# experimental-design/everest

Measured on AMD Instinct MI355X. Metric: QnehviStrategy.ask() candidates/sec + GP posterior ms, n=512 d=6 m=5, higher is better.
Workload: dtype f64; 1 GPU; full QnehviStrategy.ask() of BASELINE configs[3] (config 4): DTLZ2(d=6,m=5), n_train=512, S=256 MC samples, 1024 raw Sobol candidates + 20 L-BFGS-B restarts, q=1; value = (raw + optimiser evaluations x batch) / ask wall time, SURVEY.md §8(d); n_train=512, d=6, m=5, mc_samples=256, raw_samples=1024, restarts=20, batch_limit=20, parallelism=1 rank

## Files before the change

everest_amd/_native.py:

```python
from __future__ import annotations

import ctypes
import os
from ctypes import POINTER, c_char_p, c_double, c_int, c_longlong, c_void_p

import torch

_HERE = os.path.dirname(os.path.abspath(__file__))
LIB_PATH = os.environ.get("EVR_LIB_PATH") or os.path.join(_HERE, "_lib", "libeverest_amd.so")

c_double_p = c_void_p
c_int_p = c_void_p


class NativeLibraryError(RuntimeError):
    pass


class EvrQnehviState(ctypes.Structure):
    _fields_ = [
        ("n", c_int), ("nb", c_int), ("S", c_int), ("m", c_int),
        ("c", c_void_p), ("ym", c_void_p), ("ys", c_void_p), ("kxx", c_void_p),
        ("zq", c_void_p), ("obj_a", c_void_p), ("obj_b", c_void_p),
        ("cell_lo", c_void_p), ("cell_hi", c_void_p), ("cell_off", c_void_p), ("max_cells", c_int),
        ("cell_keys", c_void_p), ("cell_pts", c_void_p), ("cell_rank0", c_void_p), ("pts_stride", c_int),
        ("grp_off", c_void_p), ("grp_keys", c_void_p), ("grp_rank", c_void_p), ("grp_box", c_void_p),
        ("sorted_lo", c_void_p), ("max_groups", c_int), ("scan_counters", c_void_p), ("no_h", c_int),
        ("log_hvi", c_int), ("tau_relu", c_double), ("tau_max", c_double),
    ]


class EvrQnehviModel(ctypes.Structure):
    _fields_ = [
        ("n", c_int), ("d", c_int), ("kind", c_int),
        ("Xn", c_void_p), ("lengthscales", c_void_p), ("shift", c_void_p), ("scale", c_void_p), ("M", c_void_p),
    ]


class EvrQnGeneral(ctypes.Structure):
    _fields_ = [
        ("q", c_int), ("m_obj", c_int),
        ("obj_out", c_void_p), ("obj_kind", c_void_p), ("obj_p0", c_void_p), ("obj_p1", c_void_p),
        ("n_con", c_int),
        ("con_out", c_void_p), ("con_sign", c_void_p), ("con_thr", c_void_p), ("con_eta", c_void_p),
        ("zq", c_void_p),
    ]

class EvrNei(ctypes.Structure):
    _fields_ = [
        ("log", c_int), ("tau_relu", c_double), ("tau_max", c_double), ("best", c_void_p), ("best_stride", c_int),
    ]


class EvrSobo(ctypes.Structure):
    _fields_ = [
        ("log", c_int), ("tau_relu", c_double), ("tau_max", c_double), ("best", c_void_p), ("best_stride", c_int),
        ("n_term", c_int),
        ("term_out", c_void_p), ("term_kind", c_void_p), ("term_w", c_void_p), ("term_p0", c_void_p),
        ("term_p1", c_void_p), ("term_p2", c_void_p),
        ("n_con", c_int),
        ("con_out", c_void_p), ("con_sign", c_void_p), ("con_thr", c_void_p), ("con_eta", c_void_p),
    ]


class EvrParego(ctypes.Structure):
    _fields_ = [
        ("log", c_int), ("tau_relu", c_double), ("tau_max", c_double), ("best", c_void_p), ("best_stride", c_int),
        ("alpha", c_double), ("n_term", c_int),
        ("term_out", c_void_p), ("term_kind", c_void_p), ("term_p0", c_void_p), ("term_p1", c_void_p),
        ("term_a", c_void_p), ("term_b", c_void_p),
        ("n_con", c_int),
        ("con_out", c_void_p), ("con_sign", c_void_p), ("con_thr", c_void_p), ("con_eta", c_void_p),
    ]


class EvrMult(ctypes.Structure):
    _fields_ = [
        ("log", c_int), ("tau_relu", c_double), ("tau_max", c_double), ("best", c_void_p), ("best_stride", c_int),
        ("n_fac", c_int),
        ("fac_out", c_void_p), ("fac_kind", c_void_p), ("fac_w", c_void_p), ("fac_p0", c_void_p),
        ("fac_p1", c_void_p), ("fac_p2", c_void_p),
        ("n_add", c_int),
        ("add_out", c_void_p), ("add_kind", c_void_p), ("add_w", c_void_p), ("add_p0", c_void_p),
        ("add_p1", c_void_p), ("add_p2", c_void_p),
    ]


class EvrReward(ctypes.Structure):
    _fields_ = [
        ("mode", c_int), ("ucb_scale", c_double), ("tau", c_double), ("best", c_void_p),
        ("infeasible_cost", c_double), ("n_term", c_int),
        ("term_out", c_void_p), ("term_kind", c_void_p), ("term_w", c_void_p), ("term_p0", c_void_p),
        ("term_p1", c_void_p), ("term_p2", c_void_p),
        ("n_con", c_int),
        ("con_out", c_void_p), ("con_sign", c_void_p), ("con_thr", c_void_p), ("con_eta", c_void_p),
    ]


_SIGS = {
    "evr_version": ([], c_int),
    "evr_last_error": ([], c_char_p),
    "evr_device_arch": ([c_int, c_char_p, c_int], c_int),
    "evr_stream_sync": ([c_void_p], c_int),
    "evr_kernel_matrix": ([c_void_p, c_int, c_int, c_int, c_int, c_int] + [c_void_p] * 10, c_int),
    "evr_kernel_cross_grad": ([c_void_p, c_int, c_int, c_int, c_int, c_int] + [c_void_p] * 11, c_int),
    "evr_kernel_cross_grad_workspace_doubles": ([c_int, c_int, c_int], c_longlong),
    "evr_kernel_lengthscale_grad": ([c_void_p, c_int, c_int, c_int, c_int, c_void_p, c_void_p, c_void_p,
                                     c_void_p, c_void_p], c_int),
    "evr_gp_mll_terms": ([c_void_p, c_int, c_int] + [c_void_p] * 5, c_int),
    "evr_gemm_f64": ([c_void_p, c_int, c_int, c_int, c_int, c_int, c_double, c_void_p, c_int, c_longlong,
                      c_void_p, c_int, c_longlong, c_double, c_void_p, c_int, c_longlong, c_int], c_int),
    "evr_cholesky": ([c_void_p, c_int, c_int, c_void_p, c_int, c_longlong, c_void_p, c_int, c_longlong,
                      c_double, c_int, c_void_p, c_void_p], c_int),
    "evr_cholesky_inverse": ([c_void_p, c_int, c_int, c_void_p, c_int, c_longlong, c_void_p, c_int, c_longlong,
                              c_void_p, c_int, c_longlong, c_double, c_int, c_void_p, c_void_p], c_int),
    "evr_trsm_lower":([c_void_p, c_int, c_int, c_int, c_void_p, c_int, c_longlong, c_int, c_void_p, c_int,
                        c_longlong], c_int),
    "evr_tri_inv_lower": ([c_void_p, c_int, c_int, c_void_p, c_int, c_longlong, c_void_p, c_int, c_longlong],
                          c_int),
    "evr_gp_posterior_finalize": ([c_void_p, c_int, c_int, c_int] + [c_void_p] * 8, c_int),
    "evr_gp_posterior_workspace_doubles": ([c_int, c_int, c_int], c_longlong),
    "evr_gp_posterior": ([c_void_p, c_int, c_int, c_int, c_int, c_int] + [c_void_p] * 14, c_int),
    "evr_qnehvi_samples": ([c_void_p, POINTER(EvrQnehviState), c_int, c_void_p, c_void_p, c_void_p, c_void_p],
                           c_int),
    "evr_hvi_workspace_doubles": ([POINTER(EvrQnehviState), c_int, c_int], c_longlong),
    "evr_hvi_forward": ([c_void_p, POINTER(EvrQnehviState), c_int, c_void_p, c_void_p, c_void_p, c_void_p],
                        c_int),
    "evr_mean_over_samples": ([c_void_p, c_int, c_int, c_void_p, c_void_p], c_int),
    "evr_hvi_backward": ([c_void_p, POINTER(EvrQnehviState), c_int, c_void_p, c_void_p, c_void_p, c_void_p],
                         c_int),
    "evr_qnehvi_samples_backward": ([c_void_p, POINTER(EvrQnehviState), c_int, c_void_p, c_void_p, c_void_p,
                                     c_void_p], c_int),
    "evr_pareto_mask": ([c_void_p, c_int, c_int, c_int, c_void_p, c_void_p, c_int, c_void_p, c_void_p], c_int),
    "evr_objective_affine": ([c_void_p, c_int, c_int, c_int] + [c_void_p] * 5, c_int),
    "evr_qei": ([c_void_p, c_int, c_int, c_int, c_void_p, c_double, c_double, c_double, c_double, c_void_p,
                 c_double, c_double, c_double, c_void_p, c_void_p, c_void_p], c_int),
    "evr_scale_batched":([c_void_p, c_int, c_longlong, c_void_p, c_void_p], c_int),
    "evr_add_selection": ([c_void_p, c_int, c_int, c_int, c_void_p, c_void_p, c_void_p], c_int),
    "evr_box_decompose": ([c_int, c_int, c_int, c_void_p, c_longlong, c_longlong, c_longlong, c_void_p,
                           c_void_p, c_int, POINTER(c_void_p)], c_int),
    "evr_box_decompose_approx": ([c_int, c_int, c_int, c_void_p, c_longlong, c_longlong, c_longlong, c_void_p,
                                  c_void_p, c_double, c_int, POINTER(c_void_p)], c_int),
    "evr_cells_total": ([c_void_p], c_longlong),
    "evr_cells_copy": ([c_void_p, c_void_p, c_void_p, c_void_p], c_int),
    "evr_cells_free": ([c_void_p], None),
    "evr_box_device_limits": ([c_int, c_int, c_void_p, c_void_p], c_int),
    "evr_box_device_workspace_bytes": ([c_int, c_int, c_int, c_int], c_longlong),
    "evr_box_decompose_device": ([c_void_p, c_int, c_int, c_int, c_void_p, c_void_p, c_int, c_void_p, c_void_p,
                                  c_void_p], c_int),
    "evr_box_pack_keys_device": ([c_void_p, c_int, c_int, c_int, c_int, c_void_p, c_void_p, c_int, c_void_p,
                                  c_void_p, c_void_p], c_int),
    "evr_box_kd_pipeline": ([c_void_p, c_int, c_int, c_int, c_void_p, c_void_p, c_int] + [c_void_p] * 8
                            + [c_int] + [c_void_p] * 6, c_int),
    "evr_cells_from_keys": ([c_void_p, c_int, c_int, c_int, c_void_p, c_int] + [c_void_p] * 5, c_int),
    "evr_hvi_forward_backward": ([c_void_p, POINTER(EvrQnehviState), c_int] + [c_void_p] * 6, c_int),
    "evr_hvi_restart_fb_applies": ([POINTER(EvrQnehviState), c_int], c_int),
    "evr_hvi_scan_limits": ([c_int, c_int], c_int),
    "evr_hvi_restart_fb": ([c_void_p, POINTER(EvrQnehviState), c_int] + [c_void_p] * 3, c_int),
    "evr_qnehvi_norms_rows": ([POINTER(EvrQnehviState)], c_int),
    "evr_qnehvi_project": ([c_void_p, POINTER(EvrQnehviState), c_int] + [c_void_p] * 5, c_int),
    "evr_qnehvi_project_workspace_doubles": ([POINTER(EvrQnehviState), c_int], c_longlong),
    "evr_qnehvi_samples_norms": ([c_void_p, POINTER(EvrQnehviState), c_int] + [c_void_p] * 5, c_int),
    "evr_qnehvi_project_backward": ([c_void_p, POINTER(EvrQnehviState), c_int] + [c_void_p] * 6, c_int),
    "evr_qnehvi_project_backward_workspace_doubles": ([POINTER(EvrQnehviState), c_int], c_longlong),
    "evr_qnehvi_plan_workspace_bytes": ([POINTER(EvrQnehviState), POINTER(EvrQnehviModel), c_int, c_int],
                                        c_longlong),
    "evr_qnehvi_plan_create": ([c_void_p, POINTER(EvrQnehviState), POINTER(EvrQnehviModel), c_int, c_int, c_void_p,
                               c_void_p, c_void_p, c_void_p, c_int, POINTER(c_void_p)], c_int),
    "evr_qnehvi_plan_run": ([c_void_p, c_void_p], c_int),
    "evr_qnehvi_small_applies": ([POINTER(EvrQnehviState), c_int, c_int], c_int),
    "evr_qnehvi_small_workspace_doubles": ([POINTER(EvrQnehviState), c_int, c_int, c_int], ctypes.c_longlong),
    "evr_qnehvi_small_forward": ([c_void_p, POINTER(EvrQnehviState), POINTER(EvrQnehviModel), c_int, c_void_p,
                                  c_void_p, c_void_p], c_int),
    "evr_qnehvi_small_samples": ([c_void_p, POINTER(EvrQnehviState), c_int, c_void_p, c_void_p, c_void_p, c_void_p,
                                  c_void_p], c_int),
    "evr_qnehvi_small_backward": ([c_void_p, POINTER(EvrQnehviState), POINTER(EvrQnehviModel), c_int, c_void_p,
                                   c_void_p, c_void_p, c_void_p, c_void_p, c_void_p], c_int),
    "evr_mll_plan_create": ([c_void_p, c_int, c_int, c_int, c_int, c_void_p, c_void_p, c_void_p], c_int),
    "evr_mll_plan_eval": ([c_void_p, c_void_p, c_void_p, c_void_p], c_int),
    "evr_mll_plan_destroy": ([c_void_p], None),
    "evr_mll_fit_rounds": ([c_void_p, c_void_p, c_void_p] + [c_void_p] * 7 + [c_int, c_int, c_void_p, c_void_p,
                                                                             c_void_p], c_int),
    "evr_mll_assemble": ([c_int, c_int, c_int] + [c_void_p] * 6, c_int),
    "evr_kernel_matrix_members": ([c_void_p, c_int, c_int, c_int, c_int] + [c_void_p] * 5, c_int),
    "evr_kernel_lengthscale_grad_members": ([c_void_p, c_int, c_int, c_int, c_int] + [c_void_p] * 5, c_int),
    "evr_mll_plan_create_members": ([c_void_p, c_int, c_int, c_int, c_int] + [c_void_p] * 4, c_int),
    "evr_mll_assemble_members": ([c_int, c_void_p, c_int] + [c_void_p] * 6, c_int),
    "evr_lbfgsb_advance": ([c_void_p, c_double] + [c_void_p] * 6 + [c_int, c_int], c_int),
    "evr_qnehvi_plan_eval_host": ([c_void_p, c_void_p, c_void_p, c_void_p], c_int),
    "evr_qnehvi_plan_destroy": ([c_void_p], None),
    "evr_lbfgsb_create": ([c_int, c_int, c_void_p, c_void_p, c_double, c_double, c_int, POINTER(c_void_p)], c_int),
    "evr_lbfgsb_start": ([c_void_p, c_void_p, c_void_p], c_int),
    "evr_lbfgsb_step": ([c_void_p, c_double, c_void_p, c_void_p], c_int),
    "evr_lbfgsb_stats": ([c_void_p, c_void_p, c_void_p, c_void_p, c_void_p], None),
    "evr_lbfgsb_destroy": ([c_void_p], None),
    "evr_hit_and_run": ([c_int, c_int, c_void_p, c_void_p, c_int, c_void_p, c_void_p, c_longlong, ctypes.c_ulonglong,
                         c_longlong, c_longlong, c_void_p], c_int),
    "evr_qnehvi_plan_minimize": ([c_void_p, c_void_p, c_void_p, c_void_p, c_void_p, c_int, c_int, c_double,
                                  c_double, c_int, c_int, c_void_p, c_void_p, c_void_p], c_int),
    "evr_qng_workspace_doubles": ([POINTER(EvrQnehviState), POINTER(EvrQnehviState), POINTER(EvrQnGeneral),
                                   POINTER(EvrQnehviModel), c_int, c_int], c_longlong),
    "evr_qng_eval": ([c_void_p, POINTER(EvrQnehviState), POINTER(EvrQnehviState), POINTER(EvrQnGeneral),
                      POINTER(EvrQnehviModel), c_int] + [c_void_p] * 5, c_int),
    "evr_qlog_workspace_doubles": ([POINTER(EvrQnehviState), POINTER(EvrQnehviState), POINTER(EvrQnGeneral),
                                    POINTER(EvrQnehviModel), c_int, c_int], ctypes.c_longlong),
    "evr_qlog_eval": ([c_void_p, POINTER(EvrQnehviState), POINTER(EvrQnehviState), POINTER(EvrQnGeneral),
                       POINTER(EvrQnehviModel), c_int] + [c_void_p] * 5, c_int),
    "evr_nei_scan": ([c_void_p, c_int, c_int, c_int, c_int, c_void_p, c_void_p, c_int, c_double, c_double, c_double,
                      c_double, c_void_p, c_void_p, c_void_p, c_void_p], c_int),
    "evr_qnei_workspace_doubles": ([POINTER(EvrQnehviState), POINTER(EvrQnGeneral), POINTER(EvrQnehviModel), c_int,
                                    c_int], c_longlong),
    "evr_qnei_eval": ([c_void_p, POINTER(EvrQnehviState), POINTER(EvrQnGeneral), POINTER(EvrQnehviModel),
                       POINTER(EvrNei), c_int] + [c_void_p] * 5, c_int),
    "evr_sobo_scan": ([c_void_p, c_int, c_int, c_int, c_int, POINTER(EvrSobo)] + [c_void_p] * 5, c_int),
    "evr_qsobo_workspace_doubles": ([POINTER(EvrQnehviState), POINTER(EvrQnGeneral), POINTER(EvrQnehviModel), c_int,
                                     c_int], c_longlong),
    "evr_qsobo_eval": ([c_void_p, POINTER(EvrQnehviState), POINTER(EvrQnGeneral), POINTER(EvrQnehviModel),
                        POINTER(EvrSobo), c_int] + [c_void_p] * 5, c_int),
    "evr_parego_scan": ([c_void_p, c_int, c_int, c_int, c_int, POINTER(EvrParego)] + [c_void_p] * 5, c_int),
    "evr_qparego_workspace_doubles": ([POINTER(EvrQnehviState), POINTER(EvrQnGeneral), POINTER(EvrQnehviModel),
                                       c_int, c_int], c_longlong),
    "evr_qparego_eval": ([c_void_p, POINTER(EvrQnehviState), POINTER(EvrQnGeneral), POINTER(EvrQnehviModel),
                          POINTER(EvrParego), c_int] + [c_void_p] * 5, c_int),
    "evr_mult_scan": ([c_void_p, c_int, c_int, c_int, c_int, POINTER(EvrMult)] + [c_void_p] * 5, c_int),
    "evr_qmult_workspace_doubles": ([POINTER(EvrQnehviState), POINTER(EvrQnGeneral), POINTER(EvrQnehviModel),
                                     c_int, c_int], c_longlong),
    "evr_qmult_eval": ([c_void_p, POINTER(EvrQnehviState), POINTER(EvrQnGeneral), POINTER(EvrQnehviModel),
                        POINTER(EvrMult), c_int] + [c_void_p] * 5, c_int),
    "evr_reward_scan": ([c_void_p, c_int, c_int, c_int, c_int, POINTER(EvrReward)] + [c_void_p] * 5, c_int),
    "evr_qreward_workspace_doubles": ([POINTER(EvrQnehviState), POINTER(EvrQnGeneral), POINTER(EvrQnehviModel),
                                       c_int, c_int], c_longlong),
    "evr_qreward_eval": ([c_void_p, POINTER(EvrQnehviState), POINTER(EvrQnGeneral), POINTER(EvrQnehviModel),
                          POINTER(EvrReward), c_int] + [c_void_p] * 5, c_int),
    "evr_nipv_reduce": ([c_void_p] + [c_int] * 7 + [c_void_p] * 2 + [c_int] + [c_void_p] * 13, c_int),
    "evr_mixed_kernel_matrix": ([c_void_p] + [c_int] * 6 + [c_void_p] * 7, c_int),
    "evr_mixed_kernel_param_grad": ([c_void_p] + [c_int] * 5 + [c_void_p] * 6, c_int),
    "evr_objective_general": ([c_void_p, c_int, c_int, c_int, POINTER(EvrQnGeneral)] + [c_void_p] * 4, c_int),
    "evr_objective_weights": ([c_void_p, c_int, c_int, POINTER(EvrQnGeneral)] + [c_void_p] * 3, c_int),
    "evr_cells_kd_limits": ([c_int, c_int, c_int, c_void_p], c_int),
    "evr_cells_kd_order_device": ([c_void_p, c_int, c_int, c_int, c_void_p, c_void_p, c_int] + [c_void_p] * 7,
                                  c_int),
    "evr_sobol_scramble": ([c_int, ctypes.c_ulonglong, c_void_p, c_void_p], c_int),
    "evr_sobol_scramble_range": ([c_int, ctypes.c_ulonglong, c_int, c_int, c_void_p, c_void_p], c_int),
    "evr_sobol_stream_words": ([c_int], ctypes.c_longlong),
    "evr_sobol_stream_create": ([ctypes.c_ulonglong, ctypes.c_longlong, c_void_p], c_int),
    "evr_sobol_scramble_stream": ([c_void_p, c_int, c_int, c_int, c_void_p, c_void_p], c_int),
    "evr_sobol_stream_destroy": ([c_void_p], None),
    "evr_sobol_normal": ([c_void_p, c_int, c_int, c_int, c_void_p, c_void_p, c_int, c_int, c_void_p], c_int),
}

EXPORTED_SYMBOLS = tuple(_SIGS)

_lib = None


def load() -> ctypes.CDLL:
    global _lib
    if _lib is not None:
        return _lib
    if not os.path.exists(LIB_PATH):
        raise NativeLibraryError(
            f"everest_amd native library not found at {LIB_PATH}; build it with "
            "`python -c 'import __graft_entry__ as g; g.build()'` (hipcc --offload-arch=gfx950)."
        )
    lib = ctypes.CDLL(LIB_PATH, mode=ctypes.RTLD_GLOBAL)
    for name, (args, res) in _SIGS.items():
        fn = getattr(lib, name)
        fn.argtypes = args
        fn.restype = res
    _lib = lib
    return lib


def check(status: int, what: str = ""):
    if status != 0:
        msg = load().evr_last_error().decode(errors="replace")
        raise RuntimeError(f"everest_amd {what} failed (status {status}): {msg}")


def call(name: str, *args):
    lib = load()
    check(getattr(lib, name)(*args), name)
```

everest_amd/acquisition.py:

```python
from __future__ import annotations

import ctypes
import math
import os
import warnings
from dataclasses import dataclass
from typing import Optional, Sequence

import numpy as np
import torch

from . import _native, ops
from .gp import GPBatch


def sobol_base_samples(S: int, n_points: int, m: int, seed: int, device, scrambled=None) -> torch.Tensor:
    return ops.sobol_normal(S, n_points * m, seed, device, layout=1, m=m, scrambled=scrambled)


_SCRAMBLE_POOL = None


def _prefetch_scramble(dim: int, seed: int, d0: int = 0, nd: Optional[int] = None):
    global _SCRAMBLE_POOL
    nd = dim - d0 if nd is None else nd
    if nd <= 0:
        return None
    key = (int(dim), int(seed), int(d0), int(nd))
    fut = _PREFETCHED.pop(key, None)
    if fut is not None:
        return fut
    if _SCRAMBLE_POOL is None:
        from concurrent.futures import ThreadPoolExecutor

        _SCRAMBLE_POOL = ThreadPoolExecutor(max_workers=3, thread_name_prefix="evr-sobol")
    return _SCRAMBLE_POOL.submit(ops.sobol_scramble, dim, seed, d0, nd)


_PREFETCHED = {}


def prefetch_scramble(dim: int, seed: int, d0: int = 0, nd: Optional[int] = None) -> None:
    nd = dim - d0 if nd is None else nd
    key = (int(dim), int(seed), int(d0), int(nd))
    if nd <= 0 or key in _PREFETCHED:
        return
    while len(_PREFETCHED) >= 8:
        _PREFETCHED.pop(next(iter(_PREFETCHED)))
    _PREFETCHED[key] = _prefetch_scramble(dim, seed, d0, nd)


def _submit(fn, *args):
    global _SCRAMBLE_POOL
    if _SCRAMBLE_POOL is None:
        from concurrent.futures import ThreadPoolExecutor

        _SCRAMBLE_POOL = ThreadPoolExecutor(max_workers=3, thread_name_prefix="evr-sobol")
    return _SCRAMBLE_POOL.submit(fn, *args)


def _prefetch_from_stream(fut_stream, dim: int, d0: int = 0, nd: Optional[int] = None):
    nd = dim - d0 if nd is None else nd
    if nd <= 0:
        return None
    return _submit(lambda: fut_stream.result().scramble(dim, d0, nd))


def _result(fut):
    return None if fut is None else fut.result()


def _host_threads() -> int:
    v = os.environ.get("EVR_HOST_THREADS") or os.environ.get("OMP_NUM_THREADS")
    try:
        return max(1, int(v)) if v else min(16, os.cpu_count() or 1)
    except ValueError:
        return 1


def _single_cell(ref: torch.Tensor, S: int, m: int) -> ops.Cells:
    dev = ref.device
    return ops.Cells(torch.arange(S + 1, dtype=torch.int32, device=dev), np.ones(S, dtype=np.int64), m,
                     lo=ref.unsqueeze(0).repeat(S, 1).contiguous(),
                     hi=torch.full((S, m), math.inf, dtype=torch.float64, device=dev))


def _decompose(O: torch.Tensor, ref: torch.Tensor, box_device=None, kd_scan=None, num_threads=None,
               alpha: float = 0.0):
    m, P, _ = O.shape
    dev = O.device
    approx = alpha > 0.0 and m > 2
    if approx and box_device:
        raise ValueError("the device box decomposition is exact only (alpha = 0)")
    if not approx and (box_device if box_device is not None else
                       ops.box_device_supported(P, m) and ops.hvi_scan_supported(P + m, m)):
        kd_built = False
        try:
            if kd_scan is False or os.environ.get("EVR_BOX_PIPELINE", "1") == "0":
                cells = ops.box_decompose_device(O, ref)
            else:
                cells, kd_built = ops.box_decompose_kd_device(O, ref, want_kd=True)
        except ops.BoxCapacityError as e:
            if box_device:
                raise
            warnings.warn(f"{e}; using the exact host partition", RuntimeWarning)
            cells = None
        if cells is not None:
            path = "device"
            if kd_built:
                path = "device+kd"
            elif kd_scan if kd_scan is not None else ops.kd_supported(cells):
                ops.cells_kd_order(cells)
                path = "device+kd"
            elif kd_scan is None:
                warnings.warn(f"{int(cells.counts.max())} cells in one sample exceed the sparse kd scan's limit; "
                              "using the dense tiled scan (~10x slower)", RuntimeWarning)
            return cells, path
    elif not approx and box_device is None:
        warnings.warn(f"{P} points x {m} objectives exceed the device box decomposition's limits; "
                      "using the host partition", RuntimeWarning)
    mask, _ = ops.pareto_mask(O, ref, dedup=True)
    lo, hi, off = ops.box_decompose(O.cpu().numpy(), ref.cpu().numpy(), mask.cpu().numpy(),
                                    num_threads or _host_threads(), layout="jis", alpha=alpha if approx else 0.0)
    f64 = dict(dtype=torch.float64, device=dev)
    return ops.Cells(torch.as_tensor(off, dtype=torch.int32, device=dev), np.diff(off), m,
                     lo=torch.as_tensor(lo, **f64), hi=torch.as_tensor(hi, **f64)), \
        ("host-approx" if approx else "host")


_BOX_POOL = None
_SIDE_STREAMS = {}


def _decompose_async(O: torch.Tensor, ref: torch.Tensor, *args):
    global _BOX_POOL
    if os.environ.get("EVR_BOX_OVERLAP", "1") == "0" or not O.is_cuda:
        res = _decompose(O, ref, *args)
        return lambda: res
    dev = O.device
    main = torch.cuda.current_stream(dev)
    side = _SIDE_STREAMS.get(dev)
    if side is None:
        side = _SIDE_STREAMS[dev] = torch.cuda.Stream(dev)
    ready = torch.cuda.Event()
    ready.record(main)
    O.record_stream(side)
    ref.record_stream(side)
    if _BOX_POOL is None:
        from concurrent.futures import ThreadPoolExecutor

        _BOX_POOL = ThreadPoolExecutor(max_workers=1, thread_name_prefix="evr-box")

    def job():
        with torch.cuda.device(dev), torch.cuda.stream(side):
            side.wait_event(ready)
            return _decompose(O, ref, *args)

    fut = _BOX_POOL.submit(job)

    def join():
        cells, path = fut.result()
        main.wait_stream(side)
        ts = [cells.off, cells.lo, cells.hi, cells.keys, cells.pts, cells.rank0]
        if cells.kd is not None:
            kd = cells.kd
            ts += [kd.goff, kd.keys, kd.rank, kd.box, kd.sorted_lo]
        for t in ts:
            if isinstance(t, torch.Tensor) and t.is_cuda:
                t.record_stream(main)
        return cells, path

    return join


def _make_spec(m: int, obj_a, obj_b, objective, constraints) -> ops.GeneralSpec:
    if objective is None:
        a = np.asarray(obj_a, dtype=np.float64).reshape(-1)
        b = np.asarray(obj_b, dtype=np.float64).reshape(-1)
        if a.shape[0] != m or b.shape[0] != m:
            raise ValueError(f"obj_a / obj_b need one entry per model output ({m})")
        objective = [(j, ops.OBJ_AFFINE, a[j], b[j]) for j in range(m)]
    return ops.GeneralSpec(m, objective, constraints or ())


def _fast_affine(spec: ops.GeneralSpec, m: int, dev):
    f64 = dict(dtype=torch.float64, device=dev)
    if spec.affine_identity:
        return (torch.tensor([o[2] for o in spec.objectives], **f64),
                torch.tensor([o[3] for o in spec.objectives], **f64))
    return torch.ones(m, **f64), torch.zeros(m, **f64)


@dataclass
class ConstructionStats:
    n_train: int
    n_base: int
    total_cells: int
    max_cells: int
    prune_probs: Optional[np.ndarray] = None


class _BoxHviAcqf:

    @property
    def ref_point(self) -> torch.Tensor:
        return self.ref

    @property
    def constraints(self) -> list:
        return list(self.spec.constraints)

    @property
    def eta(self) -> Optional[torch.Tensor]:
        cs = self.spec.constraints
        if not cs:
            return None
        e = torch.tensor([c[3] for c in cs], dtype=torch.float64)
        return e[0] if len(set(c[3] for c in cs)) == 1 else e

    def _use_log_scan(self, tau_relu: float, tau_max: float):
        if not (tau_relu > 0 and tau_max > 0):
            raise ValueError("tau_relu and tau_max must be positive")
        lo, hi = self.cells.explicit()

        def logify(src):
            st = _native.EvrQnehviState.from_buffer_copy(src)
            st.cell_lo, st.cell_hi = lo.data_ptr(), hi.data_ptr()
            st.log_hvi, st.tau_relu, st.tau_max = 1, float(tau_relu), float(tau_max)
            return st
        self._log_cells = (lo, hi)
        self.state_scan = logify(self.state_scan)
        self.state = logify(self.state)
        if self.spec.affine_identity:
            self.state_model = self.state
        self.tau_relu, self.tau_max = float(tau_relu), float(tau_max)
        self.log_acqf = True
        self._plans = {}

    @property
    def supports_plan(self) -> bool:
        return self.spec.affine_identity and self._pending_rows() is None

    def _init_general(self, spec: ops.GeneralSpec, cells, nk: int, nb_rows: int, no_h: bool = False):
        gp, m = self.gp, self.m
        self.spec = spec
        self._zq_cache = {}
        if spec.affine_identity:
            self.state_model = self.state_scan = self.state
        else:
            ones = torch.ones(max(m, spec.m_obj), dtype=torch.float64, device=self.dev)
            self._dummy = (ones, torch.zeros_like(ones))
            self.state_model = ops.make_state(nk, nb_rows, self.S, m, gp.const, gp.ym, gp.ys, gp.kxx, self.zq,
                                              ones, ones, cells, no_h=no_h)
            self.state_scan = ops.make_state(nk, nb_rows, self.S, spec.m_obj, ones, ones, ones, ones, self.zq,
                                             ones, ones, cells, no_h=no_h)

    def _zq(self, q: int) -> torch.Tensor:
        z = self._zq_cache.get(q)
        if z is None:
            z = self._draw_zq(q).to(dtype=torch.float64, device=self.dev).reshape(self.S, q, self.m).contiguous()
            self._zq_cache[q] = z
        return z

    def set_new_point_samples(self, q: int, z: torch.Tensor):
        self._zq_cache[int(q)] = z.to(dtype=torch.float64, device=self.dev).reshape(self.S, q, self.m).contiguous()

    def _pending_rows(self) -> Optional[torch.Tensor]:
        return None

    def _general(self, X: torch.Tensor, backward: bool, gout: Optional[torch.Tensor] = None):
        b, q, d = X.shape
        Xp = self._pending_rows()
        qq = q
        if Xp is not None:
            X = torch.cat([X, Xp.unsqueeze(0).expand(b, Xp.shape[0], d)], 1)
            qq = X.shape[1]
        if qq > ops.QNG_MAX_Q:
            raise ValueError(f"joint batch of {qq} points (q + pending) exceeds the device limit of {ops.QNG_MAX_Q} "
                             f"(the inclusion-exclusion runs over all 2^q - 1 subsets)")
        g = self.spec.struct(qq, self._zq(qq))
        ev = ops.qlog_eval if getattr(self, "log_acqf", False) else ops.qng_eval
        acq, dX = ev(self.state_model, self.state_scan, g, self.model, X.reshape(b * qq, d).contiguous(),
                     backward, gout)
        if dX is not None:
            dX = dX.view(b, qq, d)[:, :q].contiguous()
        return acq, dX

    def _device_tensors(self):
        out, seen = [], set()

        def walk(v, depth=0):
            if isinstance(v, torch.Tensor):
                if v.device.type == "cuda" and id(v) not in seen:
                    seen.add(id(v))
                    out.append(v)
            elif depth >= 4 or id(v) in seen:
                return
            elif isinstance(v, (list, tuple)):
                for x in v:
                    walk(x, depth + 1)
            elif isinstance(v, dict):
                for x in v.values():
                    walk(x, depth + 1)
            elif type(v).__module__.startswith("everest_amd") and hasattr(v, "__dict__"):
                seen.add(id(v))
                for k, x in vars(v).items():
                    if k not in ("_torch_acqs", "_plans"):
                        walk(x, depth + 1)
        walk(self)
        return out

    def _torch_acq(self, q: int, fast: bool):
        from . import torch_ops

        torch_ops.load()
        cache = self.__dict__.setdefault("_torch_acqs", {})
        acq = cache.get(fast)
        if acq is None:
            def raw(st):
                return torch.frombuffer(bytearray(bytes(st)), dtype=torch.uint8)
            stm = self.state if fast else self.state_model
            sth = self.state if fast else self.state_scan
            acq = torch.classes.everest_amd.QnehviAcq(raw(stm), raw(sth), raw(self.model), bool(fast),
                                                      bool(getattr(self, "log_acqf", False)), self._device_tensors())
            cache[fast] = acq
        done = self.__dict__.setdefault("_torch_general_q", set())
        if not fast and q not in done:
            spec = self.spec
            oo, ok, p0, p1 = spec._arrs
            cons = spec.constraints
            co = torch.tensor([c[0] for c in cons], dtype=torch.int32)
            cs, ct, ce = (torch.tensor([c[k] for c in cons], dtype=torch.float64) for k in (1, 2, 3))
            acq.set_general(int(q), torch.from_numpy(oo), torch.from_numpy(ok), torch.from_numpy(p0),
                            torch.from_numpy(p1), co, cs, ct, ce, self._zq(q))
            done.add(q)
        return acq

    def __call__(self, X: torch.Tensor) -> torch.Tensor:
        from .torch_ops import QnehviFunction

        X3, _ = self._split(X)
        if self._fast(X3):
            return QnehviFunction.apply(X3[:, 0].contiguous(), self._torch_acq(1, True))
        Xp = self._pending_rows()
        if Xp is not None:
            X3 = torch.cat([X3, Xp.unsqueeze(0).expand(X3.shape[0], Xp.shape[0], X3.shape[2])], 1)
        if X3.shape[1] > ops.QNG_MAX_Q:
            raise ValueError(f"joint batch of {X3.shape[1]} points (q + pending) exceeds the device limit of "
                             f"{ops.QNG_MAX_Q} (the inclusion-exclusion runs over all 2^q - 1 subsets)")
        return QnehviFunction.apply(X3.contiguous(), self._torch_acq(X3.shape[1], False))

    def _split(self, X: torch.Tensor):
        X = X.to(device=self.dev, dtype=torch.float64)
        if X.dim() == 2:
            return X.unsqueeze(1), True
        if X.dim() != 3:
            raise ValueError(f"candidates must be b x d or b x q x d, got {tuple(X.shape)}")
        return X, False

    def _fast(self, X3: torch.Tensor) -> bool:
        return X3.shape[1] == 1 and self.supports_plan and self._pending_rows() is None

    def plan(self, b: int, backward: bool) -> ops.QnehviPlan:
        if not self.supports_plan:
            raise NotImplementedError("the native plan covers q = 1 with affine objectives on every output")
        key = (int(b), bool(backward))
        p = self._plans.get(key)
        if p is None:
            if len(self._plans) >= 8:
                self._plans.pop(next(iter(self._plans)))
            p = ops.QnehviPlan(self.state, self.model, int(b), bool(backward), self.dev,
                               graph=os.environ.get("EVR_GRAPH", "1") != "0")
            self._plans[key] = p
        return p

    def forward(self, X: torch.Tensor, return_cache: bool = False):
        if return_cache:
            return self.forward_ops(X, return_cache=True)
        X3, _ = self._split(X)
        if not self._fast(X3):
            return self._general(X3, False)[0]
        p = self.plan(X3.shape[0], False)
        p.X.copy_(X3[:, 0])
        p.run()
        return p.acq.clone()

    def forward_backward(self, X: torch.Tensor, gout: Optional[torch.Tensor] = None):
        X3, flat = self._split(X)
        if not self._fast(X3):
            acq, dX = self._general(X3, True, gout)
            return acq, (dX[:, 0] if flat else dX)
        if gout is not None:
            acq, dX = self.forward_backward_ops(X3[:, 0], gout)
            return acq, (dX if flat else dX.unsqueeze(1))
        p = self.plan(X3.shape[0], True)
        p.X.copy_(X3[:, 0])
        p.run()
        return p.acq.clone(), (p.dX.clone() if flat else p.dX.clone().unsqueeze(1))

    def eval_host(self, x: np.ndarray, backward: bool):
        b = x.shape[0]
        if x.ndim == 2 and self.supports_plan and self._pending_rows() is None:
            out = self.plan(b, backward).run_host(x)
            acq = out[:b].copy()
            return acq, (out[b:].reshape(b, -1).copy() if backward else None)
        Xt = torch.as_tensor(x, dtype=torch.float64, device=self.dev)
        if backward:
            a, g = self.forward_backward(Xt)
            return a.cpu().numpy(), g.cpu().numpy()
        return self.forward(Xt).cpu().numpy(), None

    def _cross(self, X: torch.Tensor) -> torch.Tensor:
        gp = self.gp
        return ops.kernel_matrix(self.Xk, X, gp.ls, gp.kind, shift2=gp.lo, scale2=gp.inv_range)

    def forward_ops(self, X: torch.Tensor, return_cache: bool = False):
        X = X.to(device=self.dev, dtype=torch.float64).contiguous()
        b = X.shape[0]
        Kx = self._cross(X)
        R, P = ops.qnehvi_project(self.state, self.M, Kx, b)
        G, L22, flags = ops.qnehvi_samples_norms(self.state, R, P, b)
        acq = ops.hvi_forward(self.state, G, b, flags)
        if return_cache:
            return acq, (X, R, G, L22, flags)
        return acq

    def forward_backward_ops(self, X: torch.Tensor, gout: Optional[torch.Tensor] = None):
        X = X.to(device=self.dev, dtype=torch.float64).contiguous()
        b = X.shape[0]
        Kx = self._cross(X)
        R, P = ops.qnehvi_project(self.state, self.M, Kx, b)
        G, L22, flags = ops.qnehvi_samples_norms(self.state, R, P, b)
        acq, dG = ops.hvi_forward_backward(self.state, G, b, flags, gout)
        dKx = ops.qnehvi_project_backward(self.state, self.M, R, L22, dG, b)
        gp = self.gp
        dX = ops.kernel_cross_grad(self.Xk, X, gp.ls, dKx, gp.kind, shift2=gp.lo, scale2=gp.inv_range)
        return acq, dX


class QNEHVI(_BoxHviAcqf):

    def __init__(self, gp: GPBatch, X_train_raw: np.ndarray, X_baseline_raw: np.ndarray, ref_point, obj_a, obj_b,
                 S: int = 512, sampler_seed: int = 0, prune_baseline: bool = True, prune_seed: int = 0,
                 prune_samples: int = 2048, max_frac: float = 1.0, z_prune: Optional[torch.Tensor] = None,
                 z_base_full: Optional[torch.Tensor] = None, z_new_full: Optional[torch.Tensor] = None,
                 num_threads: Optional[int] = None, box_device: Optional[bool] = None,
                 kd_scan: Optional[bool] = None, X_pending_raw: Optional[np.ndarray] = None,
                 root: Optional[str] = None, objective=None, constraints=(), alpha: float = 0.0):
        dev = gp.device
        self.gp = gp
        self.dev = dev
        m = gp.B
        n = gp.n
        self.m, self.n, self.S = m, n, int(S)
        f64 = dict(dtype=torch.float64, device=dev)
        spec = _make_spec(m, obj_a, obj_b, objective, constraints)
        self.spec = spec
        self.ref = torch.as_tensor(np.asarray(ref_point, dtype=np.float64), **f64)
        if self.ref.numel() != spec.m_obj:
# ... 944 lines not shown
```

everest_amd/csrc/box_device.hip:

```cpp
#include <algorithm>
#include <cmath>
#include <cstdlib>

#include "common.hpp"
#include "../../include/everest_amd.h"

namespace evr {

constexpr int BD_THREADS = 1024;
constexpr unsigned long long BD_DEAD = ~0ull;
constexpr int BD_LDS_BYTES = 160 * 1024 - 2048;
constexpr int BD_STG = 256;

struct BdLayout {
  long long cap;
  int n, m;
  size_t off_lub, off_buf, off_aidx, off_pts, off_inv0, off_nf, bytes;
};

static BdLayout bd_layout(int S, int n, int m, int cap) {
  BdLayout L;
  L.cap = cap;
  L.n = n;
  L.m = m;
  size_t o = 0;
  auto take = [&](size_t b) {
    size_t r = o;
    o += (b + 255) & ~(size_t)255;
    return r;
  };
  L.off_lub = take(sizeof(unsigned long long) * (size_t)S * cap);
  L.off_buf = take(sizeof(unsigned long long) * (size_t)S * cap);
  L.off_aidx = take(sizeof(int) * (size_t)S * cap);
  L.off_pts = take(sizeof(double) * (size_t)S * (n + m) * m);
  L.off_inv0 = take(sizeof(int) * (size_t)S * (n + m));
  L.off_nf = take(sizeof(int) * (size_t)S);
  L.bytes = o;
  return L;
}

static size_t bd_lds_fixed(int n, int m) {
  return sizeof(double) * ((size_t)n * m + (size_t)(n + m) * m) + sizeof(int) * (size_t)(4 * n + 2 * m + 8);
}

template <typename Ptr>
__device__ void bd_bitonic(Ptr a, int P2) {
  for (int k = 2; k <= P2; k <<= 1) {
    for (int j = k >> 1; j > 0; j >>= 1) {
      for (int i = threadIdx.x; i < P2; i += BD_THREADS) {
        const int l = i ^ j;
        if (l > i) {
          const unsigned long long x = a[i], y = a[l];
          const bool up = (i & k) == 0;
          if ((x > y) == up) {
            a[i] = y;
            a[l] = x;
          }
        }
      }
      __syncthreads();
    }
  }
}

template <int M, bool LS>
__global__ __launch_bounds__(BD_THREADS) void bd_build_kernel(int S, int n, const double* __restrict__ obj,
                                                              const double* __restrict__ ref, int cap, int sortcap,
                                                              unsigned char* __restrict__ ws, BdLayout Lo,
                                                              int* __restrict__ counts, int* __restrict__ status,
                                                              int* hmap) {
  using K = CellKey<M>;
  extern __shared__ __align__(16) unsigned char smem[];
  const int s = blockIdx.x, tid = threadIdx.x;
  double* raw = (double*)smem;
  double* pt = raw + (size_t)n * M;
  int* flag = (int*)(pt + (size_t)(n + M) * M);
  int* pos = flag + n;
  int* inv0 = pos + n;
  int* rank = inv0 + n + M;
  unsigned long long* sbuf = (unsigned long long*)(((uintptr_t)(rank + n + M) + 15) & ~(uintptr_t)15);
  unsigned long long* stg = sbuf + sortcap;
  int* astg = (int*)(stg + BD_STG);
  __shared__ int sh_nf, sh_nA, sh_nNew, sh_cnt, sh_err;

  unsigned long long* lub = LS ? sbuf : (unsigned long long*)(ws + Lo.off_lub) + (size_t)s * cap;
  unsigned long long* buf = (unsigned long long*)(ws + Lo.off_buf) + (size_t)s * cap;
  int* aidx = (int*)(ws + Lo.off_aidx) + (size_t)s * cap;
  double* gpts = (double*)(ws + Lo.off_pts) + (size_t)s * (n + M) * M;
  int* ginv0 = (int*)(ws + Lo.off_inv0) + (size_t)s * (n + M);

  for (int e = tid; e < n * M; e += BD_THREADS) {
    const int i = e / M, j = e - i * M;
    raw[e] = -obj[((size_t)j * n + i) * S + s];
  }
  if (tid == 0) sh_err = 0;
  __syncthreads();
  for (int i = tid; i < n; i += BD_THREADS) {
    bool keep = true;
#pragma unroll
    for (int j = 0; j < M; ++j) keep &= raw[i * M + j] < -ref[j];
    for (int k = 0; k < n && keep; ++k) {
      if (k == i) continue;
      bool cand = true, le = true, lt = false, eq = true;
#pragma unroll
      for (int j = 0; j < M; ++j) {
        const double v = raw[k * M + j], w = raw[i * M + j];
        cand &= v < -ref[j];
        le &= v <= w;
        lt |= v < w;
        eq &= v == w;
      }
      if (cand && ((le && lt) || (eq && k < i))) keep = false;
    }
    flag[i] = keep ? 1 : 0;
  }
  __syncthreads();
  if (tid == 0) {
    int c = 0;
    for (int i = 0; i < n; ++i) {
      pos[i] = c;
      c += flag[i];
    }
    sh_nf = c;
  }
  __syncthreads();
  const int nf = sh_nf;
  for (int e = tid; e < n * M; e += BD_THREADS) {
    const int i = e / M;
    if (flag[i]) pt[pos[i] * M + (e - i * M)] = raw[e];
  }
  for (int e = tid; e < M * M; e += BD_THREADS) {
    const int k = e / M, j = e - k * M;
    pt[(nf + k) * M + j] = (j == k) ? -ref[k] : -INFINITY;
  }
  __syncthreads();
  for (int i = tid; i <= nf; i += BD_THREADS) {
    const double v = pt[i * M];
    int r = 0;
    for (int k = 0; k <= nf; ++k) {
      const double w = pt[k * M];
      r += (w > v) || (w == v && k < i);
    }
    inv0[r] = i;
    rank[i] = r;
  }
  __syncthreads();

  int Kend = 1, holes = 0;
  if (tid == 0) {
    unsigned long long k0 = 0;
    k0 = K::set(k0, 0, rank[nf]);
    for (int j = 1; j < M; ++j) k0 = K::set(k0, j, nf + j);
    lub[0] = k0;
  }
  __syncthreads();
  for (int p = 0; p < nf; ++p) {
    double z[M];
#pragma unroll
    for (int j = 0; j < M; ++j) z[j] = pt[p * M + j];
    if (tid == 0) {
      sh_nA = 0;
      sh_nNew = 0;
    }
    __syncthreads();
    for (int u = tid; u < Kend; u += BD_THREADS) {
      const unsigned long long key = lub[u];
      if (key == BD_DEAD) continue;
      bool dom = pt[inv0[K::field(key, 0)] * M] > z[0];
#pragma unroll
      for (int j = 1; j < M; ++j) dom &= pt[K::field(key, j) * M + j] > z[j];
      if (dom) {
        const int k = atomicAdd(&sh_nA, 1);
        if (LS && k < BD_STG) astg[k] = u;
        else aidx[k] = u;
      }
    }
    __syncthreads();
    const int nA = sh_nA;
    for (int t = tid; t < nA * M; t += BD_THREADS) {
      const int a = t / M, j = t - a * M;
      const unsigned long long key = lub[(LS && a < BD_STG) ? astg[a] : aidx[a]];
      double zmax = -INFINITY;
#pragma unroll
      for (int k = 0; k < M; ++k) {
        if (k == j) continue;
        const int pk = (k == 0) ? inv0[K::field(key, 0)] : K::field(key, k);
        zmax = fmax(zmax, pt[pk * M + j]);
      }
      if (z[j] >= zmax) {
        const int slot = atomicAdd(&sh_nNew, 1);
        if (slot < cap) {
          const unsigned long long nk = K::set(key, j, j == 0 ? rank[p] : p);
          if (LS && slot < BD_STG) stg[slot] = nk;
          else buf[slot] = nk;
        }
      }
    }
    __syncthreads();
    const int nNew = sh_nNew;
    if (Kend + (nNew > nA ? nNew - nA : 0) > cap || nNew > cap) {
      if (tid == 0) sh_err = 1;
      break;
    }
    const int top = nNew > nA ? nNew : nA;
    for (int i = tid; i < top; i += BD_THREADS) {
      const bool st = LS && i < BD_STG;
      if (i < nNew) {
        const int dst = (i < nA) ? (st ? astg[i] : aidx[i]) : Kend + (i - nA);
        lub[dst] = st ? stg[i] : buf[i];
      } else {
        lub[st ? astg[i] : aidx[i]] = BD_DEAD;
      }
    }
    if (nNew > nA) Kend += nNew - nA;
    else holes += nA - nNew;
    __syncthreads();
    if (holes > 256 && holes * 4 > Kend) {
      if (tid == 0) sh_cnt = 0;
      __syncthreads();
      for (int u = tid; u < Kend; u += BD_THREADS) {
        const unsigned long long key = lub[u];
        if (key != BD_DEAD) buf[atomicAdd(&sh_cnt, 1)] = key;
      }
      __syncthreads();
      const int cnt = sh_cnt;
      for (int u = tid; u < cnt; u += BD_THREADS) lub[u] = buf[u];
      Kend = cnt;
      holes = 0;
      __syncthreads();
    }
  }
  __syncthreads();
  if (sh_err) {
    if (tid == 0) {
      status[s] = 1;
      counts[s] = 0;
      if (hmap) {
        hmap[s] = 0;
        hmap[S + s] = 1;
      }
    }
    return;
  }

  if (tid == 0) sh_cnt = 0;
  __syncthreads();
  for (int u = tid; u < Kend; u += BD_THREADS) {
    const unsigned long long key = lub[u];
    if (key == BD_DEAD) continue;
    int P[M];
    P[0] = inv0[K::field(key, 0)];
#pragma unroll
    for (int j = 1; j < M; ++j) P[j] = K::field(key, j);
    bool ok = true;
#pragma unroll
    for (int j = 1; j < M; ++j) {
      double lo = -INFINITY;
#pragma unroll
      for (int k = 0; k < j; ++k) lo = fmax(lo, pt[P[k] * M + j]);
      ok &= pt[P[j] * M + j] > lo;
    }
    if (ok) buf[atomicAdd(&sh_cnt, 1)] = key;
  }
  __syncthreads();
  const int C = sh_cnt;
  int P2 = 1;
  while (P2 < C) P2 <<= 1;
  if (P2 <= sortcap) {
    for (int i = tid; i < P2; i += BD_THREADS) sbuf[i] = (i < C) ? buf[i] : BD_DEAD;
    __syncthreads();
    wg_bitonic<unsigned long long, BD_THREADS>(sbuf, P2);
    for (int i = tid; i < C; i += BD_THREADS) buf[i] = sbuf[i];
  } else {
    for (int i = C + tid; i < P2; i += BD_THREADS) buf[i] = BD_DEAD;
    __syncthreads();
    bd_bitonic(buf, P2);
  }
  for (int e = tid; e < (nf + M) * M; e += BD_THREADS) gpts[e] = pt[e];
  for (int r = tid; r <= nf; r += BD_THREADS) ginv0[r] = inv0[r];
  if (tid == 0) {
    counts[s] = C;
    status[s] = 0;
    ((int*)(ws + Lo.off_nf))[s] = nf;
    if (hmap) {
      hmap[s] = C;
      hmap[S + s] = 0;
    }
  }
}

template <int M>
__global__ __launch_bounds__(256) void cells_from_keys_kernel(int stride, const int* __restrict__ off,
                                                              const unsigned long long* __restrict__ keys,
                                                              const double* __restrict__ pts,
                                                              const int* __restrict__ rank0, double* __restrict__ lo,
                                                              double* __restrict__ hi) {
  using K = CellKey<M>;
  const int s = blockIdx.y;
  const int i = blockIdx.x * 256 + threadIdx.x;
  const int c0 = off[s], C = off[s + 1] - c0;
  if (i >= C) return;
  double l[M], h[M];
  K::decode(keys[c0 + i], pts + (size_t)s * stride * M, rank0 + (size_t)s * stride, l, h);
  const size_t o = (size_t)(c0 + i) * M;
#pragma unroll
  for (int j = 0; j < M; ++j) {
    lo[o + j] = l[j];
    hi[o + j] = h[j];
  }
}

template <int M>
__global__ __launch_bounds__(256) void bd_pack_keys_kernel(int S, int n, int cap, const unsigned char* __restrict__ ws,
                                                           BdLayout Lo, const int* __restrict__ off,
                                                           unsigned long long* __restrict__ keys,
                                                           double* __restrict__ pts, int* __restrict__ rank0) {
  const int s = blockIdx.y;
  const int i = blockIdx.x * 256 + threadIdx.x;
  const int c0 = off[s], C = off[s + 1] - c0;
  if (i < C) keys[c0 + i] = ((const unsigned long long*)(ws + Lo.off_buf))[(size_t)s * cap + i];
  if (blockIdx.x == 0) {
    const size_t np = (size_t)(n + M);
    const double* gp = (const double*)(ws + Lo.off_pts) + s * np * M;
    const int* gi = (const int*)(ws + Lo.off_inv0) + s * np;
    const size_t nv = (size_t)((const int*)(ws + Lo.off_nf))[s] + M;
    for (size_t e = threadIdx.x; e < np * M; e += 256) pts[s * np * M + e] = e < nv * M ? gp[e] : INFINITY;
    for (size_t e = threadIdx.x; e < np; e += 256) rank0[s * np + e] = e + M <= nv ? gi[e] : 0;
  }
}

}

using namespace evr;

#define EVR_BD_SWITCH(m, MACRO)                                                       \
  switch (m) {                                                                        \
    case 1: MACRO(1); break;                                                          \
    case 2: MACRO(2); break;                                                          \
    case 3: MACRO(3); break;                                                          \
    case 4: MACRO(4); break;                                                          \
    case 5: MACRO(5); break;                                                          \
    case 6: MACRO(6); break;                                                          \
    case 7: MACRO(7); break;                                                          \
    case 8: MACRO(8); break;                                                          \
    default: EVR_CHECK(false, "box decomposition: m=%d not supported (1..8)", m);     \
  }

extern "C" {

int evr_box_device_limits(int n, int m, int* max_points_out, long long* lds_bytes_out) {
  EVR_CHECK(m >= 1 && m <= 8 && n >= 0, "evr_box_device_limits: bad arguments");
  const long long idx_limit = (1ll << bd_field_bits(m)) - 2 - m;
  const size_t fixed = bd_lds_fixed(n, m);
  if (max_points_out) *max_points_out = (int)std::min<long long>(idx_limit, 1 << 20);
  if (lds_bytes_out) *lds_bytes_out = (long long)fixed;
  return (n <= idx_limit && fixed + 16 + 8 * 64 <= (size_t)BD_LDS_BYTES) ? 0 : 3;
}

long long evr_box_device_workspace_bytes(int S, int n, int m, int cap) {
  if (S < 1 || n < 0 || m < 1 || cap < 1) return 0;
  return (long long)bd_layout(S, n, m, cap).bytes;
}

static int box_decompose_launch(void* stream, int S, int n, int m, const double* obj, const double* ref, int cap,
                                void* work, int* counts, int* status, int* hmap);

int evr_box_decompose_device(void* stream, int S, int n, int m, const double* obj, const double* ref, int cap,
                             void* work, int* counts, int* status) {
  return box_decompose_launch(stream, S, n, m, obj, ref, cap, work, counts, status, nullptr);
}

static int box_decompose_launch(void* stream, int S, int n, int m, const double* obj, const double* ref, int cap,
                                void* work, int* counts, int* status, int* hmap) {
  EVR_CHECK(S >= 1 && n >= 1 && m >= 1 && m <= 8 && obj && ref && work && counts && status,
            "evr_box_decompose_device: bad arguments");
  EVR_CHECK(cap >= 2 && (cap & (cap - 1)) == 0, "evr_box_decompose_device: cap must be a power of two");
  EVR_CHECK(evr_box_device_limits(n, m, nullptr, nullptr) == 0,
            "evr_box_decompose_device: n=%d points x m=%d exceed the device limits", n, m);
  const BdLayout Lo = bd_layout(S, n, m, cap);
  const size_t fixed = bd_lds_fixed(n, m) + 16;
  auto sort_cap = [&](size_t fx) {
    int c = 1;
    while ((size_t)(c * 2) * 8 + fx <= (size_t)BD_LDS_BYTES && c * 2 <= cap) c *= 2;
    return c;
  };
  const size_t fixed_ls = fixed + (size_t)BD_STG * (8 + 4);
  const char* ev = std::getenv("EVR_BD_LDS");
  const bool ls = sort_cap(fixed_ls) >= cap && !(ev && ev[0] == '0');
  const int sortcap = ls ? cap : sort_cap(fixed);
  const size_t lds = (ls ? fixed_ls : fixed) + (size_t)sortcap * 8;
  hipStream_t s = (hipStream_t)stream;
#define L2(MM, LS_)                                                                                          \
  do {                                                                                                       \
    EVR_HIP(hipFuncSetAttribute((const void*)bd_build_kernel<MM, LS_>,                                      \
                                hipFuncAttributeMaxDynamicSharedMemorySize, (int)lds));                      \
    bd_build_kernel<MM, LS_><<<S, BD_THREADS, lds, s>>>(S, n, obj, ref, cap, sortcap, (unsigned char*)work, \
                                                        Lo, counts, status, hmap);                           \
  } while (0)
#define L(MM)            \
  if (ls) L2(MM, true);  \
  else L2(MM, false)
  EVR_BD_SWITCH(m, L);
#undef L
#undef L2
  EVR_LAUNCH_CHECK();
  return 0;
}

int evr_cells_from_keys(void* stream, int S, int m, int stride, const int* off, int max_cells,
                        const unsigned long long* keys, const double* pts, const int* rank0, double* lo,
                        double* hi) {
  EVR_CHECK(S >= 1 && m >= 1 && m <= 8 && stride > m && off && keys && pts && rank0 && lo && hi,
            "evr_cells_from_keys: bad arguments");
  if (max_cells <= 0) return 0;
  dim3 grid(cdiv(max_cells, 256), S);
  hipStream_t s = (hipStream_t)stream;
#define L(MM) cells_from_keys_kernel<MM><<<grid, 256, 0, s>>>(stride, off, keys, pts, rank0, lo, hi)
  EVR_BD_SWITCH(m, L);
#undef L
  EVR_LAUNCH_CHECK();
  return 0;
}

int evr_box_pack_keys_device(void* stream, int S, int n, int m, int cap, const void* work, const int* off,
                             int max_cells, unsigned long long* keys, double* pts, int* rank0) {
  EVR_CHECK(S >= 1 && n >= 1 && m >= 1 && m <= 8 && work && off && keys && pts && rank0,
            "evr_box_pack_keys_device: bad arguments");
  const BdLayout Lo = bd_layout(S, n, m, cap);
  dim3 grid(std::max(1, cdiv(max_cells, 256)), S);
  hipStream_t s = (hipStream_t)stream;
#define L(MM) \
  bd_pack_keys_kernel<MM><<<grid, 256, 0, s>>>(S, n, cap, (const unsigned char*)work, Lo, off, keys, pts, rank0)
  EVR_BD_SWITCH(m, L);
#undef L
  EVR_LAUNCH_CHECK();
  return 0;
}


int evr_box_kd_pipeline(void* stream, int S, int n, int m, const double* obj, const double* ref, int cap,
                        void* work, int* counts_dev, int* status_dev, int* off_dev, int* goff_dev,
                        unsigned long long* keys, double* pts, int* rank0, int want_kd, unsigned long long* okeys,
                        unsigned short* ork, unsigned short* ogb, double* osv, int* counts_host, int* info) {
  EVR_CHECK(S >= 1 && counts_dev && status_dev && off_dev && goff_dev && keys && pts && rank0 && counts_host &&
                info && (!want_kd || (okeys && ork && ogb && osv)),
            "evr_box_kd_pipeline: bad arguments");
  hipStream_t s = (hipStream_t)stream;
  thread_local int* stage = nullptr;
  thread_local int* stage_d = nullptr;
  thread_local size_t stage_n = 0;
  thread_local int stage_dev = -1;
  thread_local hipEvent_t copied = nullptr;
  if (copied) EVR_HIP(hipEventSynchronize(copied));
  int dev = 0;
  EVR_HIP(hipGetDevice(&dev));
  const size_t need = (size_t)4 * S + 2;
  if (stage_n < need || stage_dev != dev) {
    if (copied) {
      (void)hipEventDestroy(copied);
      copied = nullptr;
    }
    if (stage) (void)hipHostFree(stage);
    stage = stage_d = nullptr;
    stage_n = 0;
    stage_dev = -1;
    EVR_HIP(hipHostMalloc((void**)&stage, sizeof(int) * need, hipHostMallocMapped | hipHostMallocCoherent));
    EVR_HIP(hipHostGetDevicePointer((void**)&stage_d, stage, 0));
    stage_n = need;
    stage_dev = dev;
  }
  if (!copied) EVR_HIP(hipEventCreateWithFlags(&copied, hipEventDisableTiming));
  int* hc = stage;
  int* hs = stage + S;
  int* hoff = stage + 2 * S;
  int* hgoff = hoff + S + 1;
  if (int rc = box_decompose_launch(stream, S, n, m, obj, ref, cap, work, counts_dev, status_dev, stage_d)) return rc;
  EVR_HIP(hipStreamSynchronize(s));
  info[0] = info[1] = info[2] = 0;
  int maxc = 0;
  for (int i = 0; i < S; ++i) {
    counts_host[i] = hc[i];
    if (hs[i]) info[0] = 1;
    maxc = std::max(maxc, hc[i]);
  }
  info[2] = maxc;
  if (info[0]) return 0;
  long long c = 0, g = 0;
  for (int i = 0; i < S; ++i) {
    hoff[i] = (int)c;
    hgoff[i] = (int)g;
    c += hc[i];
    g += (hc[i] + 15) / 16;
  }
  hoff[S] = (int)c;
  hgoff[S] = (int)g;
  EVR_CHECK(c <= (long long)S * cap && c < 0x7FFFFFFFLL, "evr_box_kd_pipeline: %lld cells exceed the capacity", c);
  const int* moff = stage_d + 2 * S;
  const int* mgoff = moff + S + 1;
  if (int rc = evr_box_pack_keys_device(stream, S, n, m, cap, work, moff, maxc, keys, pts, rank0)) return rc;
  const int stride = n + m;
  if (want_kd && evr_cells_kd_limits(stride, m, maxc, nullptr) == 0) {
    if (int rc = evr_cells_kd_order_device(stream, S, m, stride, moff, mgoff, maxc, keys, pts, rank0, okeys, ork,
                                           ogb, osv))
      return rc;
    info[1] = 1;
  }
  EVR_HIP(hipMemcpyAsync(off_dev, hoff, sizeof(int) * (S + 1), hipMemcpyHostToDevice, s));
  EVR_HIP(hipMemcpyAsync(goff_dev, hgoff, sizeof(int) * (S + 1), hipMemcpyHostToDevice, s));
  EVR_HIP(hipEventRecord(copied, s));
  return 0;
}

}
```

everest_amd/csrc/qnehvi.hip:

```cpp
#include <algorithm>
#include <cstdlib>
#include <string>
#include "common.hpp"
#include "../../include/everest_amd.h"

namespace evr {

template <int BX>
__global__ __launch_bounds__(256) void qn_samples_kernel(int n, int nb, int S, int nh, int m, int b,
                                                         const double* __restrict__ R,
                                                         const double* __restrict__ cc,
                                                         const double* __restrict__ ym,
                                                         const double* __restrict__ ys,
                                                         const double* __restrict__ kxx,
                                                         const double* __restrict__ zq,
                                                         const double* __restrict__ oa,
                                                         const double* __restrict__ ob, double* __restrict__ G,
                                                         double* __restrict__ L22, int* __restrict__ flags) {
  constexpr int RY = 256 / BX;
  __shared__ double red[2][RY][BX];
  const int j = blockIdx.y;
  const int cx = threadIdx.x % BX, ry = threadIdx.x / BX;
  const int c = blockIdx.x * BX + cx;
  const bool live = c < b;
  const long long Rr = (long long)n + nb + nh + 1;
  const double* Rj = R + (size_t)j * Rr * b;
  double ssv = 0.0, ssw = 0.0;
  if (live) {
    for (int i = ry; i < n; i += RY) {
      const double v = Rj[(size_t)i * b + c];
      ssv = fma(v, v, ssv);
    }
    for (int i = n + ry; i < n + nb; i += RY) {
      const double v = Rj[(size_t)i * b + c];
      ssw = fma(v, v, ssw);
    }
  }
  red[0][ry][cx] = ssv;
  red[1][ry][cx] = ssw;
  __syncthreads();
  ssv = 0.0;
  ssw = 0.0;
#pragma unroll
  for (int g = 0; g < RY; ++g) {
    ssv += red[0][g][cx];
    ssw += red[1][g][cx];
  }
  if (!live) return;
  const double a = Rj[(size_t)(n + nb + nh) * b + c];
  const double s = ys[j];
  const double mu = ym[j] + s * (cc[j] + a);
  const double var = s * s * (kxx[j] - ssv);
  const double br = var - ssw;
  double l22 = nan("");
  int flag = 1;
  if (!isnan(br)) {
    for (int t = 0; t <= 6; ++t) {
      const double jit = (t == 0) ? 0.0 : 1e-8 * pow(10.0, (double)(t - 1));
      if (br + jit > 0.0) {
        l22 = sqrt(br + jit);
        flag = 0;
        break;
      }
    }
  }
  if (ry == 0) {
    L22[(size_t)j * b + c] = l22;
    flags[(size_t)j * b + c] = flag;
  }
  const double A = oa[j], B0 = ob[j];
  const double* h = Rj + (size_t)(n + nb) * b + c;
  for (int si = ry; si < S; si += RY) {
    const double y = (nh ? mu + h[(size_t)si * b] : mu) + l22 * zq[(size_t)si * m + j];
    G[((size_t)si * m + j) * b + c] = fma(A, y, B0);
  }
}

__global__ void mean_over_samples_kernel(int S, int b, const double* __restrict__ partial, double* __restrict__ acq) {
  const int c = blockIdx.x * blockDim.x + threadIdx.x;
  if (c >= b) return;
  double s = 0.0;
  for (int i = 0; i < S; ++i) s += partial[(size_t)i * b + c];
  acq[c] = s / (double)S;
}

template <int BX>
__global__ __launch_bounds__(256) void qn_samples_bwd_kernel(int n, int nb, int S, int nh, int m, int b,
                                                             const double* __restrict__ R,
                                                             const double* __restrict__ ys,
                                                             const double* __restrict__ zq,
                                                             const double* __restrict__ oa,
                                                             const double* __restrict__ L22,
                                                             const double* __restrict__ dG, double* __restrict__ gR) {
  constexpr int RY = 256 / BX;
  __shared__ double red[2][RY][BX];
  const int j = blockIdx.y;
  const int cx = threadIdx.x % BX, ry = threadIdx.x / BX;
  const int c = blockIdx.x * BX + cx;
  const bool live = c < b;
  const long long Rr = (long long)n + nb + nh + 1;
  const double* Rj = R + (size_t)j * Rr * b;
  double* gj = gR + (size_t)j * Rr * b;
  const double A = oa[j];
  double dmu = 0.0, dl = 0.0;
  if (live) {
    for (int si = ry; si < S; si += RY) {
      const double dy = A * dG[((size_t)si * m + j) * b + c];
      dmu += dy;
      dl = fma(dy, zq[(size_t)si * m + j], dl);
      if (nh) gj[(size_t)(n + nb + si) * b + c] = dy;
    }
  }
  red[0][ry][cx] = dmu;
  red[1][ry][cx] = dl;
  __syncthreads();
  dmu = 0.0;
  dl = 0.0;
#pragma unroll
  for (int g = 0; g < RY; ++g) {
    dmu += red[0][g][cx];
    dl += red[1][g][cx];
  }
  if (!live) return;
  const double s = ys[j];
  if (ry == 0) gj[(size_t)(n + nb + nh) * b + c] = s * dmu;
  const double l22 = L22[(size_t)j * b + c];
  const double dbr = dl / (2.0 * l22);
  const double dssv = -s * s * dbr;
  const double dssw = -dbr;
  for (int i = ry; i < n; i += RY) gj[(size_t)i * b + c] = 2.0 * Rj[(size_t)i * b + c] * dssv;
  for (int i = n + ry; i < n + nb; i += RY) gj[(size_t)i * b + c] = 2.0 * Rj[(size_t)i * b + c] * dssw;
}

template <int M>
__global__ void pareto_kernel(int S, int n, const double* __restrict__ O, const double* __restrict__ ref,
                              int dedup, unsigned char* __restrict__ mask, int* __restrict__ counts) {
  const int s = blockIdx.x * blockDim.x + threadIdx.x;
  const int i = blockIdx.y;
  if (s >= S) return;
  double yi[M];
  bool better = true;
#pragma unroll
  for (int j = 0; j < M; ++j) {
    yi[j] = O[((size_t)j * n + i) * S + s];
    better &= yi[j] > ref[j];
  }
  bool nd = better;
  for (int k = 0; k < n && nd; ++k) {
    if (k == i) continue;
    bool ge = true, gt = false, eq = true;
#pragma unroll
    for (int j = 0; j < M; ++j) {
      const double v = O[((size_t)j * n + k) * S + s];
      ge &= v >= yi[j];
      gt |= v > yi[j];
      eq &= v == yi[j];
    }
    if (ge && gt) nd = false;
    if (dedup && eq && k < i) nd = false;
  }
  if (mask) mask[(size_t)s * n + i] = nd ? 1 : 0;
  if (counts && nd) atomicAdd(&counts[i], 1);
}

template <int M>
__global__ __launch_bounds__(256) void pareto_lds_kernel(int S, int n, int SB, const double* __restrict__ O,
                                                         const double* __restrict__ ref, int dedup,
                                                         unsigned char* __restrict__ mask, int* __restrict__ counts) {
  extern __shared__ double pts[];
  const int s0 = blockIdx.x * SB, sb = min(SB, S - s0);
  const int tot = M * n * sb;
  for (int e = threadIdx.x; e < tot; e += 256) {
    const int j = e / (n * sb), rem = e - j * n * sb, k = rem / sb, ss = rem - k * sb;
    pts[((size_t)ss * n + k) * M + j] = O[((size_t)j * n + k) * S + s0 + ss];
  }
  double rj[M];
#pragma unroll
  for (int j = 0; j < M; ++j) rj[j] = ref[j];
  __syncthreads();
  for (int p = threadIdx.x; p < sb * n; p += 256) {
    const int ss = p / n, i = p - ss * n;
    const double* P = pts + (size_t)ss * n * M;
    double yi[M];
    bool better = true;
#pragma unroll
    for (int j = 0; j < M; ++j) {
      yi[j] = P[i * M + j];
      better &= yi[j] > rj[j];
    }
    bool nd = better;
    constexpr int U = 8;
    for (int k0 = 0; k0 < n && nd; k0 += U) {
      double v[U][M];
#pragma unroll
      for (int u = 0; u < U; ++u)
#pragma unroll
        for (int j = 0; j < M; ++j) v[u][j] = (k0 + u < n) ? P[(k0 + u) * M + j] : 0.0;
#pragma unroll
      for (int u = 0; u < U; ++u) {
        const int k = k0 + u;
        if (k >= n || k == i) continue;
        bool ge = true, gt = false, eq = true;
#pragma unroll
        for (int j = 0; j < M; ++j) {
          ge &= v[u][j] >= yi[j];
          gt |= v[u][j] > yi[j];
          eq &= v[u][j] == yi[j];
        }
        if (ge && gt) nd = false;
        if (dedup && eq && k < i) nd = false;
      }
    }
    if (mask) mask[(size_t)(s0 + ss) * n + i] = nd ? 1 : 0;
    if (counts && nd) atomicAdd(&counts[i], 1);
  }
}

template <int M>
__global__ __launch_bounds__(256) void pareto_f32_kernel(int S, int n, int npad, int SB, const double* __restrict__ O,
                                                         const double* __restrict__ ref, int dedup,
                                                         unsigned char* __restrict__ mask, int* __restrict__ counts) {
  extern __shared__ double pts[];
  float* ptf = reinterpret_cast<float*>(pts + (((size_t)SB * n * M + 1) & ~(size_t)1));
  const int s0 = blockIdx.x * SB, sb = min(SB, S - s0);
  const int tot = M * n * sb;
  for (int e = threadIdx.x; e < tot; e += 256) {
    const int j = e / (n * sb), rem = e - j * n * sb, k = rem / sb, ss = rem - k * sb;
    const double v = O[((size_t)j * n + k) * S + s0 + ss];
    pts[((size_t)ss * n + k) * M + j] = v;
    ptf[((size_t)ss * M + j) * npad + k] = (float)v;
  }
  for (int e = threadIdx.x; e < sb * M * (npad - n); e += 256) {
    const int r = e / (npad - n), k = n + (e - r * (npad - n));
    ptf[(size_t)r * npad + k] = -INFINITY;
  }
  double rj[M];
#pragma unroll
  for (int j = 0; j < M; ++j) rj[j] = ref[j];
  __syncthreads();
  for (int p = threadIdx.x; p < sb * n; p += 256) {
    const int ss = p / n, i = p - ss * n;
    const double* P = pts + (size_t)ss * n * M;
    const float* F = ptf + (size_t)ss * M * npad;
    double yi[M];
    float yf[M];
    bool better = true;
#pragma unroll
    for (int j = 0; j < M; ++j) {
      yi[j] = P[i * M + j];
      yf[j] = (float)yi[j];
      better &= yi[j] > rj[j];
    }
    bool nd = better;
    for (int k0 = 0; k0 < n && nd; k0 += 8) {
      float4 va[M], vb[M];
#pragma unroll
      for (int j = 0; j < M; ++j) {
        va[j] = *reinterpret_cast<const float4*>(F + (size_t)j * npad + k0);
        vb[j] = *reinterpret_cast<const float4*>(F + (size_t)j * npad + k0 + 4);
      }
      bool ge8[8];
#pragma unroll
      for (int u = 0; u < 8; ++u) ge8[u] = k0 + u != i && k0 + u < n;
#pragma unroll
      for (int j = 0; j < M; ++j) {
        ge8[0] &= va[j].x >= yf[j]; ge8[1] &= va[j].y >= yf[j];
        ge8[2] &= va[j].z >= yf[j]; ge8[3] &= va[j].w >= yf[j];
        ge8[4] &= vb[j].x >= yf[j]; ge8[5] &= vb[j].y >= yf[j];
        ge8[6] &= vb[j].z >= yf[j]; ge8[7] &= vb[j].w >= yf[j];
      }
      unsigned int cand = 0;
#pragma unroll
      for (int u = 0; u < 8; ++u) cand |= (unsigned int)ge8[u] << u;
      while (cand) {
        const int u = __builtin_ctz(cand);
        cand &= cand - 1;
        const int k = k0 + u;
        bool ge = true, gt = false, eq = true;
#pragma unroll
        for (int j = 0; j < M; ++j) {
          const double v = P[k * M + j];
          ge &= v >= yi[j];
          gt |= v > yi[j];
          eq &= v == yi[j];
        }
        if ((ge && gt) || (dedup && eq && k < i)) {
          nd = false;
          cand = 0;
        }
      }
    }
    if (mask) mask[(size_t)(s0 + ss) * n + i] = nd ? 1 : 0;
    if (counts && nd) atomicAdd(&counts[i], 1);
  }
}

__global__ void qei_kernel(int n, int b, int S, const double* __restrict__ R, double cc, double ym, double ys,
                           double kxx, const double* __restrict__ z, double oa, double ob, double best_f,
                           double* __restrict__ acq, double* __restrict__ gR, int* __restrict__ flags) {
  const int c = blockIdx.x * blockDim.x + threadIdx.x;
  if (c >= b) return;
  double ss = 0.0;
  for (int i = 0; i < n; ++i) {
    const double v = R[(size_t)i * b + c];
    ss = fma(v, v, ss);
  }
  const double mu = ym + ys * (cc + R[(size_t)n * b + c]);
  const double var = ys * ys * (kxx - ss);
  double sd = nan("");
  int flag = 1;
  if (!isnan(var)) {
    for (int t = 0; t <= 3; ++t) {
      const double jit = (t == 0) ? 0.0 : 1e-8 * pow(10.0, (double)(t - 1));
      if (var + jit > 0.0) {
        sd = sqrt(var + jit);
        flag = 0;
        break;
      }
    }
  }
  double tot = 0.0, dmu = 0.0, dsd = 0.0;
  for (int s = 0; s < S; ++s) {
    const double imp = oa * (mu + sd * z[s]) + ob - best_f;
    if (imp > 0.0) {
      tot += imp;
      dmu += oa;
      dsd += oa * z[s];
    }
  }
  acq[c] = tot / S;
  flags[c] = flag;
  if (gR) {
    dmu /= S;
    dsd /= S;
    const double dvar = dsd / (2.0 * sd);
    const double dss = -ys * ys * dvar;
    for (int i = 0; i < n; ++i) gR[(size_t)i * b + c] = 2.0 * R[(size_t)i * b + c] * dss;
    gR[(size_t)n * b + c] = ys * dmu;
  }
}

__global__ void scale_batched_kernel(long long per, const double* __restrict__ alpha, double* __restrict__ X) {
  const long long e = (long long)blockIdx.x * blockDim.x + threadIdx.x;
  if (e >= per) return;
  X[(size_t)blockIdx.y * per + e] *= alpha[blockIdx.y];
}

__global__ void add_selection_kernel(int nb, int n, const int* __restrict__ idx, const double* __restrict__ val,
                                     double* __restrict__ E) {
  const int r = blockIdx.x * blockDim.x + threadIdx.x;
  if (r >= nb) return;
  const int b = blockIdx.y;
  E[((size_t)b * nb + r) * n + idx[r]] += val ? val[b] : 1.0;
}

__global__ void objective_affine_kernel(int m, int n, int S, const double* __restrict__ Y, const double* __restrict__ mu,
                                        const double* __restrict__ a, const double* __restrict__ bb,
                                        double* __restrict__ O) {
  const long long e = (long long)blockIdx.x * blockDim.x + threadIdx.x;
  const long long tot = (long long)m * n * S;
  if (e >= tot) return;
  const int j = (int)(e / ((long long)n * S));
  const int i = (int)((e / S) % n);
  const double mv = mu ? mu[(size_t)j * n + i] : 0.0;
  O[e] = fma(a[j], Y[e] + mv, bb[j]);
}

}

using namespace evr;

#define EVR_DISPATCH_M(m, MACRO)                                                      \
  switch (m) {                                                                        \
    case 1: MACRO(1); break;                                                          \
    case 2: MACRO(2); break;                                                          \
    case 3: MACRO(3); break;                                                          \
    case 4: MACRO(4); break;                                                          \
    case 5: MACRO(5); break;                                                          \
    case 6: MACRO(6); break;                                                          \
    case 7: MACRO(7); break;                                                          \
    case 8: MACRO(8); break;                                                          \
    default: EVR_CHECK(false, "number of objectives m=%d not supported (1..8)", m);   \
  }

extern "C" {

int evr_qnehvi_samples(void* stream, const evr_qnehvi_state* st, int b, const double* R, double* G, double* L22,
                       int* flags) {
  EVR_CHECK(st && st->m >= 1 && st->S >= 1 && st->n >= 1 && st->nb >= 0, "evr_qnehvi_samples: bad state");
  if (b == 0) return 0;
  hipStream_t s = (hipStream_t)stream;
  if (b <= 256) {
    dim3 grid(cdiv(b, 16), st->m);
    qn_samples_kernel<16><<<grid, 256, 0, s>>>(st->n, st->nb, st->S, qn_nh(st), st->m, b, R, st->c, st->ym, st->ys, st->kxx,
                                               st->zq, st->obj_a, st->obj_b, G, L22, flags);
  } else {
    dim3 grid(cdiv(b, 64), st->m);
    qn_samples_kernel<64><<<grid, 256, 0, s>>>(st->n, st->nb, st->S, qn_nh(st), st->m, b, R, st->c, st->ym, st->ys, st->kxx,
                                               st->zq, st->obj_a, st->obj_b, G, L22, flags);
  }
  EVR_LAUNCH_CHECK();
  return 0;
}

int evr_mean_over_samples(void* stream, int S, int b, const double* partial, double* acq) {
  if (b == 0) return 0;
  mean_over_samples_kernel<<<cdiv(b, 256), 256, 0, (hipStream_t)stream>>>(S, b, partial, acq);
  EVR_LAUNCH_CHECK();
  return 0;
}

int evr_qnehvi_samples_backward(void* stream, const evr_qnehvi_state* st, int b, const double* R, const double* L22,
                                const double* dG, double* gR) {
  EVR_CHECK(st && st->m >= 1, "evr_qnehvi_samples_backward: bad state");
  if (b == 0) return 0;
  hipStream_t s = (hipStream_t)stream;
  if (b <= 256) {
    dim3 grid(cdiv(b, 16), st->m);
    qn_samples_bwd_kernel<16><<<grid, 256, 0, s>>>(st->n, st->nb, st->S, qn_nh(st), st->m, b, R, st->ys, st->zq, st->obj_a,
                                                   L22, dG, gR);
  } else {
    dim3 grid(cdiv(b, 64), st->m);
    qn_samples_bwd_kernel<64><<<grid, 256, 0, s>>>(st->n, st->nb, st->S, qn_nh(st), st->m, b, R, st->ys, st->zq, st->obj_a,
                                                   L22, dG, gR);
  }
  EVR_LAUNCH_CHECK();
  return 0;
}

int evr_pareto_mask(void* stream, int S, int n, int m, const double* O, const double* ref, int dedup,
                    unsigned char* mask, int* counts) {
  EVR_CHECK(S >= 1 && n >= 0, "evr_pareto_mask: bad sizes");
  if (n == 0) return 0;
  hipStream_t s = (hipStream_t)stream;
  constexpr size_t kLds = 96 * 1024;
  const size_t per = (size_t)n * m * sizeof(double);
  constexpr int f32_filter = 1;
  const int npad = (n + 7) & ~7;
  const size_t per2 = (size_t)n * m * sizeof(double) + (size_t)npad * m * sizeof(float);
  constexpr size_t kLds2 = 78 * 1024;
  if (f32_filter && per2 <= kLds2) {
    const int SB = (int)std::min<size_t>(4, kLds2 / per2);
    const size_t bytes = (((size_t)SB * n * m + 1) & ~(size_t)1) * sizeof(double) + (size_t)SB * npad * m * sizeof(float);
#define L(MM)                                                                                            \
  do {                                                                                                   \
    EVR_HIP(hipFuncSetAttribute((const void*)pareto_f32_kernel<MM>,                                       \
                                hipFuncAttributeMaxDynamicSharedMemorySize, (int)bytes));                \
    pareto_f32_kernel<MM><<<cdiv(S, SB), 256, bytes, s>>>(S, n, npad, SB, O, ref, dedup, mask, counts);  \
  } while (0)
    EVR_DISPATCH_M(m, L);
#undef L
  } else if (per <= kLds) {
    const int SB = (int)std::min<size_t>(4, kLds / per);
    const size_t bytes = per * SB;
#define L(MM)                                                                                            \
  do {                                                                                                   \
    EVR_HIP(hipFuncSetAttribute((const void*)pareto_lds_kernel<MM>,                                       \
                                hipFuncAttributeMaxDynamicSharedMemorySize, (int)bytes));                \
    pareto_lds_kernel<MM><<<cdiv(S, SB), 256, bytes, s>>>(S, n, SB, O, ref, dedup, mask, counts);       \
  } while (0)
    EVR_DISPATCH_M(m, L);
#undef L
  } else {
    dim3 grid(cdiv(S, 64), n);
#define L(MM) pareto_kernel<MM><<<grid, 64, 0, s>>>(S, n, O, ref, dedup, mask, counts)
    EVR_DISPATCH_M(m, L);
#undef L
  }
  EVR_LAUNCH_CHECK();
  return 0;
}

int evr_qei(void* stream, int n, int b, int S, const double* R, double c, double ym, double ys, double kxx,
            const double* z, double obj_a, double obj_b, double best_f, double* acq, double* gR, int* flags) {
  EVR_CHECK(n >= 1 && S >= 1, "evr_qei: bad sizes");
  if (b == 0) return 0;
  qei_kernel<<<cdiv(b, 256), 256, 0, (hipStream_t)stream>>>(n, b, S, R, c, ym, ys, kxx, z, obj_a, obj_b, best_f,
                                                            acq, gR, flags);
  EVR_LAUNCH_CHECK();
  return 0;
}

int evr_scale_batched(void* stream, int B, long long per, const double* alpha, double* X) {
  if (per == 0) return 0;
  dim3 grid(cdiv(per, 256), B);
  scale_batched_kernel<<<grid, 256, 0, (hipStream_t)stream>>>(per, alpha, X);
  EVR_LAUNCH_CHECK();
  return 0;
}

int evr_add_selection(void* stream, int B, int nb, int n, const int* idx, const double* val, double* E) {
  if (nb == 0) return 0;
  dim3 grid(cdiv(nb, 256), B);
  add_selection_kernel<<<grid, 256, 0, (hipStream_t)stream>>>(nb, n, idx, val, E);
  EVR_LAUNCH_CHECK();
  return 0;
}

int evr_objective_affine(void* stream, int m, int n, int S, const double* Y, const double* mu, const double* a,
                         const double* b, double* O) {
  const long long tot = (long long)m * n * S;
  if (tot == 0) return 0;
  objective_affine_kernel<<<cdiv(tot, 256), 256, 0, (hipStream_t)stream>>>(m, n, S, Y, mu, a, b, O);
  EVR_LAUNCH_CHECK();
  return 0;
}

}
```

everest_amd/ops.py:

```python
from __future__ import annotations

import ctypes
import math
import os
import warnings
from typing import Optional, Tuple

import numpy as np
import torch

from . import _native
from ._native import EvrQnehviState, EvrQnGeneral, call

KERNELS = {"rbf": 0, "matern05": 1, "matern15": 2, "matern25": 3}
KIND_BY_NU = {0.5: 1, 1.5: 2, 2.5: 3}


class NotPSDError(RuntimeError):
    """Raised when the jitter ladder of psd_safe_cholesky is exhausted ([upstream]
    linear_operator NotPSDError, caught by fit_gpytorch_mll's retries)."""


QNG_MAX_Q = 12

# ... 866 lines not shown
        d = int(model.d)
        self.b, self.d, self.backward = int(b), d, bool(backward)
        self.X = torch.zeros(b, d, dtype=torch.float64, device=device)
        self.out = torch.empty(b * (1 + d), dtype=torch.float64, device=device)
        nbytes = lib.evr_qnehvi_plan_workspace_bytes(ctypes.byref(st), ctypes.byref(model), b, int(backward))
        self.work = torch.empty(max(nbytes, 1), dtype=torch.uint8, device=device)
        self.acq = self.out[:b]
        self.dX = self.out[b:].view(b, d)
        self.host = torch.zeros(b * (1 + d), dtype=torch.float64)
        h = ctypes.c_void_p()
        call("evr_qnehvi_plan_create", _stream(), ctypes.byref(st), ctypes.byref(model), b, int(backward),
             self.X.data_ptr(), self.work.data_ptr(), self.acq.data_ptr(),
             self.dX.data_ptr() if backward else None, int(graph), ctypes.byref(h))
        self._h = h
        self._lib = lib

    def run(self):
        call("evr_qnehvi_plan_run", _stream(), self._h)

    def run_host(self, x: np.ndarray) -> np.ndarray:
        xh = np.ascontiguousarray(x, dtype=np.float64).reshape(self.b, self.d)
        out = self.host.numpy()
        call("evr_qnehvi_plan_eval_host", _stream(), self._h, xh.ctypes.data, out.ctypes.data)
        return out

    def minimize(self, x0: np.ndarray, lb: np.ndarray, ub: np.ndarray, maxiter: int, maxfun: int = 15000,
                 maxcor: int = 10, ftol: float = 2.220446049250313e-09, gtol: float = 1e-5, maxls: int = 20):
        if not self.backward:
            raise ValueError("minimize needs a backward plan")
        n = self.b * self.d
        f64 = lambda a: np.ascontiguousarray(np.asarray(a, dtype=np.float64).reshape(n))
        x0, lb, ub = f64(x0), f64(lb), f64(ub)
        x = np.empty(n)
        acq = np.empty(self.b)
        info = np.zeros(4, dtype=np.int32)
        rc = self._lib.evr_qnehvi_plan_minimize(_stream(), self._h, x0.ctypes.data, lb.ctypes.data, ub.ctypes.data,
                                                int(maxiter), int(maxfun), ftol / float(np.finfo(float).eps),
                                                float(gtol), int(maxcor), int(maxls), x.ctypes.data,
                                                acq.ctypes.data, info.ctypes.data)
        if rc == 7:
            raise NotPSDError(self._lib.evr_last_error().decode(errors="replace"))
        _native.check(rc, "evr_qnehvi_plan_minimize")
        return x, acq, info.tolist()

    def __del__(self):
        h = getattr(self, "_h", None)
        if h is not None and h.value:
            self._lib.evr_qnehvi_plan_destroy(h)
            self._h = None


def _hvi_work(st: EvrQnehviState, b: int, backward: bool, device) -> torch.Tensor:
    n = _native.load().evr_hvi_workspace_doubles(ctypes.byref(st), b, int(backward))
    return torch.empty(max(1, n), dtype=torch.float64, device=device)


def hvi_forward(st: EvrQnehviState, G: torch.Tensor, b: int, flags: Optional[torch.Tensor] = None) -> torch.Tensor:
    acq = torch.empty(b, dtype=torch.float64, device=G.device)
    work = _hvi_work(st, b, False, G.device)
    call("evr_hvi_forward", _stream(), ctypes.byref(st), b, G.data_ptr(), _p(flags), work.data_ptr(),
         acq.data_ptr())
    return acq


def mean_over_samples(partial: torch.Tensor):
    S, b = partial.shape
    acq = torch.empty(b, dtype=torch.float64, device=partial.device)
    call("evr_mean_over_samples", _stream(), S, b, partial.data_ptr(), acq.data_ptr())
    return acq


def hvi_backward(st: EvrQnehviState, G: torch.Tensor, gout: Optional[torch.Tensor], b: int):
    dG = torch.empty_like(G)
    if gout is not None:
        gout = _dev(gout, "gout")
    work = _hvi_work(st, b, True, G.device)
    call("evr_hvi_backward", _stream(), ctypes.byref(st), b, G.data_ptr(), _p(gout), work.data_ptr(),
         dG.data_ptr())
    return dG


def hvi_forward_backward(st: EvrQnehviState, G: torch.Tensor, b: int, flags: Optional[torch.Tensor] = None,
                         gout: Optional[torch.Tensor] = None):
    acq = torch.empty(b, dtype=torch.float64, device=G.device)
    dG = torch.empty_like(G)
    if gout is not None:
        gout = _dev(gout, "gout")
    work = _hvi_work(st, b, True, G.device)
    call("evr_hvi_forward_backward", _stream(), ctypes.byref(st), b, G.data_ptr(), _p(flags), _p(gout),
         work.data_ptr(), acq.data_ptr(), dG.data_ptr())
    return acq, dG


def hvi_restart_fb_applies(st: EvrQnehviState, b: int) -> bool:
    return bool(_native.load().evr_hvi_restart_fb_applies(ctypes.byref(st), int(b)))


def hvi_restart_fb(st: EvrQnehviState, G: torch.Tensor, b: int):
    S = int(st.S)
    sval = torch.empty(S, b, dtype=torch.float64, device=G.device)
    dG = torch.empty_like(G)
    call("evr_hvi_restart_fb", _stream(), ctypes.byref(st), b, G.data_ptr(), sval.data_ptr(), dG.data_ptr())
    return sval, dG


def qnehvi_samples_backward(st: EvrQnehviState, R, L22, dG, b: int):
    gR = torch.empty_like(R)
    call("evr_qnehvi_samples_backward", _stream(), ctypes.byref(st), b, R.data_ptr(), L22.data_ptr(), dG.data_ptr(),
         gR.data_ptr())
    return gR


def pareto_mask(O: torch.Tensor, ref: torch.Tensor, dedup: bool, want_mask=True, want_counts=False):
    O, ref = _dev(O, "O"), _dev(ref, "ref")
    m, n, S = O.shape
    mask = torch.empty(S, n, dtype=torch.uint8, device=O.device) if want_mask else None
    counts = torch.zeros(n, dtype=torch.int32, device=O.device) if want_counts else None
    call("evr_pareto_mask", _stream(), S, n, m, O.data_ptr(), ref.data_ptr(), int(dedup), _p(mask), _p(counts))
    return mask, counts


def objective_affine(Y: torch.Tensor, mu: Optional[torch.Tensor], a: torch.Tensor, b: torch.Tensor):
    Y = _dev(Y, "Y")
    m, n, S = Y.shape
    O = torch.empty_like(Y)
    mu = None if mu is None else _dev(mu, "mu")
    call("evr_objective_affine", _stream(), m, n, S, Y.data_ptr(), _p(mu), _dev(a, "a").data_ptr(),
         _dev(b, "b").data_ptr(), O.data_ptr())
    return O


def qei(R: torch.Tensor, c: float, ym: float, ys: float, kxx: float, z: torch.Tensor, a: float, b: float,
        best_f: float, with_grad: bool):
    R, z = _dev(R, "R"), _dev(z, "z")
    n1, nb = R.shape
    acq = torch.empty(nb, dtype=torch.float64, device=R.device)
    gR = torch.empty_like(R) if with_grad else None
    flags = torch.empty(nb, dtype=torch.int32, device=R.device)
    call("evr_qei", _stream(), n1 - 1, nb, z.numel(), R.data_ptr(), float(c), float(ym), float(ys), float(kxx),
         z.data_ptr(), float(a), float(b), float(best_f), acq.data_ptr(), _p(gR), flags.data_ptr())
    return acq, gR, flags


def nipv_reduce(C: torch.Tensor, Vx: torch.Tensor, X: torch.Tensor, lo, inv_range, lengthscales, kind: int, noise,
                coef, v0, n: Optional[int] = None, backward: bool = False, gout: Optional[torch.Tensor] = None):
    C, Vx, X = _dev(C, "C"), _dev(Vx, "Vx"), _dev(X, "X")
    ls = _dev(lengthscales, "lengthscales")
    if X.dim() != 3 or C.dim() != 3 or Vx.dim() != 3 or ls.dim() != 2:
        raise ValueError("nipv_reduce: C, Vx and X are 3-D, lengthscales 2-D")
    b, q, d = X.shape
    B, N, bq = C.shape
    ldv = Vx.shape[1]
    n = ldv if n is None else int(n)
    if bq != b * q or Vx.shape[0] != B or Vx.shape[2] != bq or tuple(ls.shape) != (B, d) or not 1 <= n <= ldv:
        raise ValueError(f"nipv_reduce: shapes C {tuple(C.shape)} Vx {tuple(Vx.shape)} X {tuple(X.shape)} "
                         f"ls {tuple(ls.shape)} n {n}")
    lo, inv_range = _dev(lo, "lo"), _dev(inv_range, "inv_range")
    noise, coef, v0 = _dev(noise, "noise"), _dev(coef, "coef"), _dev(v0, "v0")
    if lo.numel() != d or inv_range.numel() != d or noise.numel() != B or coef.numel() != B or v0.numel() != B:
        raise ValueError("nipv_reduce: lo / inv_range need d values, noise / coef / v0 one per output")
    if gout is not None:
        if not backward:
            raise ValueError("nipv_reduce: gout weights the backward only")
        gout = _dev(gout, "gout")
        if gout.numel() != b:
            raise ValueError("nipv_reduce: gout needs one value per candidate")
    dev = C.device
    acq = torch.empty(b, dtype=torch.float64, device=dev)
    flags = torch.empty(b, dtype=torch.int32, device=dev)
    dC = torch.empty_like(C) if backward else None
    dVx = torch.empty(B, n, bq, dtype=torch.float64, device=dev) if backward else None
    dXs = torch.empty_like(X) if backward else None
    call("evr_nipv_reduce", _stream(), int(q), B, n, N, b, d, int(kind), C.data_ptr(), Vx.data_ptr(), ldv,
         X.data_ptr(), lo.data_ptr(), inv_range.data_ptr(), ls.data_ptr(), noise.data_ptr(), coef.data_ptr(),
         v0.data_ptr(), _p(gout), acq.data_ptr(), flags.data_ptr(), _p(dC), _p(dVx), _p(dXs))
    return acq, flags, dC, dVx, dXs


def scale_batched(X: torch.Tensor, alpha: torch.Tensor) -> torch.Tensor:
    if not X.is_contiguous():
        raise ValueError("scale_batched: X must be contiguous")
    B = X.shape[0]
    call("evr_scale_batched", _stream(), B, X.numel() // B, _dev(alpha, "alpha").data_ptr(), X.data_ptr())
    return X


def add_selection(E: torch.Tensor, idx: torch.Tensor, val: Optional[torch.Tensor]) -> torch.Tensor:
    B, nb, n = E.shape
    idx = _dev(idx, "idx", torch.int32)
    call("evr_add_selection", _stream(), B, nb, n, idx.data_ptr(), _p(None if val is None else _dev(val, "val")),
         E.data_ptr())
    return E


def box_device_supported(n: int, m: int) -> bool:
    return _native.load().evr_box_device_limits(int(n), int(m), None, None) == 0


def hvi_scan_supported(stride: int, m: int) -> bool:
    return _native.load().evr_hvi_scan_limits(int(stride), int(m)) == 0


class Cells:

    def __init__(self, off, counts, m, lo=None, hi=None, keys=None, pts=None, rank0=None, stride=0):
        self.off, self.counts, self.m = off, np.asarray(counts, dtype=np.int64), int(m)
        self.lo, self.hi, self.keys, self.pts, self.rank0, self.stride = lo, hi, keys, pts, rank0, int(stride)
        self.kd: Optional[KdGroups] = None

    @property
    def S(self) -> int:
        return int(self.counts.shape[0])

    @property
    def total(self) -> int:
        return int(self.counts.sum())

    @property
    def max_cells(self) -> int:
        return int(self.counts.max()) if self.S else 0

    def explicit(self) -> Tuple[torch.Tensor, torch.Tensor]:
        if self.keys is None:
            return self.lo, self.hi
        lo = torch.empty(self.total, self.m, dtype=torch.float64, device=self.off.device)
        hi = torch.empty_like(lo)
        call("evr_cells_from_keys", _stream(), self.S, self.m, self.stride, self.off.data_ptr(), self.max_cells,
             self.keys.data_ptr(), self.pts.data_ptr(), self.rank0.data_ptr(), lo.data_ptr(), hi.data_ptr())
        return lo, hi


class KdGroups:

    def __init__(self, goff, keys, rank, box, sorted_lo, max_groups):
        self.goff, self.keys, self.rank, self.box = goff, keys, rank, box
        self.sorted_lo, self.max_groups = sorted_lo, int(max_groups)


def kd_supported(cells: Cells) -> bool:
    if cells.keys is None or cells.S == 0:
        return False
    return _native.load().evr_cells_kd_limits(cells.stride, cells.m, cells.max_cells, None) == 0


def cells_kd_order(cells: Cells) -> KdGroups:
    if cells.keys is None:
        raise ValueError("cells_kd_order needs compressed cells (device box decomposition)")
    S, m, stride = cells.S, cells.m, cells.stride
    dev = cells.off.device
    ng = (cells.counts + 15) // 16
    goff_h = np.zeros(S + 1, dtype=np.int64)
    np.cumsum(ng, out=goff_h[1:])
    G = int(goff_h[-1])
    goff = torch.as_tensor(goff_h.astype(np.int32)).to(dev)
    keys = torch.empty(max(G, 1) * 16, dtype=torch.int64, device=dev)
    rank = torch.empty(max(G, 1) * m * 16, dtype=torch.int16, device=dev)
    box = torch.empty(max(G, 1) * 8, dtype=torch.int16, device=dev)
    sorted_lo = torch.empty(S, m, stride, dtype=torch.float64, device=dev)
    call("evr_cells_kd_order_device", _stream(), S, m, stride, cells.off.data_ptr(), goff.data_ptr(),
         cells.max_cells, cells.keys.data_ptr(), cells.pts.data_ptr(), cells.rank0.data_ptr(), keys.data_ptr(),
         rank.data_ptr(), box.data_ptr(), sorted_lo.data_ptr())
    cells.kd = KdGroups(goff, keys, rank, box, sorted_lo, int(ng.max()) if S else 0)
    return cells.kd


class BoxCapacityError(RuntimeError):
    """The device box decomposition needs more LUB slots than its capacity / memory bound
    (the caller falls back to the exact host partition)."""


def box_decompose_device(O: torch.Tensor, ref: torch.Tensor, cap: int = 16384, max_cap: int = 1 << 20,
                         max_workspace_bytes: int = 8 << 30) -> Cells:
    O, ref = _dev(O, "O"), _dev(ref, "ref")
    m, n, S = O.shape
    dev = O.device
    while True:
        nbytes = _native.load().evr_box_device_workspace_bytes(S, n, m, cap)
        if nbytes > max_workspace_bytes:
            raise BoxCapacityError(f"box decomposition: {cap} LUB slots x {S} samples need {nbytes} B of workspace")
        ws = torch.empty(nbytes, dtype=torch.uint8, device=dev)
        cs = torch.empty(2, S, dtype=torch.int32, device=dev)
        call("evr_box_decompose_device", _stream(), S, n, m, O.data_ptr(), ref.data_ptr(), cap, ws.data_ptr(),
             cs[0].data_ptr(), cs[1].data_ptr())
        h = cs.cpu().numpy()
        if not h[1].any():
            break
        if cap >= max_cap:
            raise BoxCapacityError(f"box decomposition: more than {max_cap} local upper bounds in one sample")
        cap *= 4
    counts = h[0].astype(np.int64)
    off_h = np.zeros(S + 1, dtype=np.int64)
    np.cumsum(counts, out=off_h[1:])
    total = int(off_h[-1])
    off = torch.as_tensor(off_h.astype(np.int32)).to(dev)
    stride = n + m
    keys = torch.empty(max(total, 1), dtype=torch.int64, device=dev)
    pts = torch.empty(S, stride, m, dtype=torch.float64, device=dev)
    rank0 = torch.empty(S, stride, dtype=torch.int32, device=dev)
    call("evr_box_pack_keys_device", _stream(), S, n, m, cap, ws.data_ptr(), off.data_ptr(),
         int(counts.max()) if S else 0, keys.data_ptr(), pts.data_ptr(), rank0.data_ptr())
    return Cells(off, counts, m, keys=keys, pts=pts, rank0=rank0, stride=stride)


def box_decompose_kd_device(O: torch.Tensor, ref: torch.Tensor, want_kd: bool = True, cap: int = 16384,
                            max_cap: int = 1 << 20, max_workspace_bytes: int = 8 << 30):
    O, ref = _dev(O, "O"), _dev(ref, "ref")
    m, n, S = O.shape
    dev = O.device
    stride = n + m
    lib = _native.load()
    counts_h = np.zeros(S, dtype=np.int32)
    info = np.zeros(3, dtype=np.int32)
    cap0 = cap
    while True:
        nbytes = lib.evr_box_device_workspace_bytes(S, n, m, cap)
        G = S * cap // 16 + S
        out_bytes = 8 * S * cap + 8 * S * stride * m + 4 * S * stride + 16 * S + 8
        if want_kd:
            out_bytes += G * 16 * 8 + G * m * 16 * 2 + G * 8 * 2 + 8 * S * m * stride
        if nbytes + out_bytes > max_workspace_bytes:
            raise BoxCapacityError(f"box decomposition: {cap} LUB slots x {S} samples need {nbytes + out_bytes} B "
                                   "of workspace and outputs")
        try:
            ws = torch.empty(nbytes, dtype=torch.uint8, device=dev)
            cs = torch.empty(2, S, dtype=torch.int32, device=dev)
            offs = torch.empty(2, S + 1, dtype=torch.int32, device=dev)
            keys = torch.empty(S * cap, dtype=torch.int64, device=dev)
            pts = torch.empty(S, stride, m, dtype=torch.float64, device=dev)
            rank0 = torch.empty(S, stride, dtype=torch.int32, device=dev)
            if want_kd:
                okeys = torch.empty(G * 16, dtype=torch.int64, device=dev)
                ork = torch.empty(G * m * 16, dtype=torch.int16, device=dev)
                ogb = torch.empty(G * 8, dtype=torch.int16, device=dev)
                osv = torch.empty(S, m, stride, dtype=torch.float64, device=dev)
            else:
                okeys = ork = ogb = osv = None
        except torch.OutOfMemoryError as e:
            raise BoxCapacityError(f"box decomposition: out of device memory at {cap} LUB slots x {S} samples") from e
        call("evr_box_kd_pipeline", _stream(), S, n, m, O.data_ptr(), ref.data_ptr(), cap, ws.data_ptr(),
             cs[0].data_ptr(), cs[1].data_ptr(), offs[0].data_ptr(), offs[1].data_ptr(), keys.data_ptr(),
             pts.data_ptr(), rank0.data_ptr(), int(bool(want_kd)), _p(okeys), _p(ork), _p(ogb), _p(osv),
             counts_h.ctypes.data, info.ctypes.data)
        if not info[0]:
            break
        if cap >= max_cap:
            raise BoxCapacityError(f"box decomposition: more than {max_cap} local upper bounds in one sample")
        cap *= 4
    counts = counts_h.astype(np.int64)
    total = int(counts.sum())
    del ws
    trim = (lambda t: t.clone()) if cap > cap0 else (lambda t: t)
    cells = Cells(offs[0], counts, m, keys=trim(keys[:max(total, 1)]), pts=pts, rank0=rank0, stride=stride)
    if info[1]:
        ng = (counts + 15) // 16
        Gu = int(ng.sum())
        cells.kd = KdGroups(offs[1], trim(okeys[:max(Gu, 1) * 16]), trim(ork[:max(Gu, 1) * m * 16]),
                            trim(ogb[:max(Gu, 1) * 8]), osv, int(ng.max()) if S else 0)
    return cells, bool(info[1])


_SOBOL_DIRECTIONS = {}


def _sobol_directions(dim: int) -> torch.Tensor:
    V = _SOBOL_DIRECTIONS.get(dim)
    if V is None:
        V = torch.zeros(dim, 30, dtype=torch.long)
        torch._sobol_engine_initialize_state_(V, dim)
        if len(_SOBOL_DIRECTIONS) > 16:
            _SOBOL_DIRECTIONS.clear()
        _SOBOL_DIRECTIONS[dim] = V
    return V


SOBOL_MAXDIM = 21201


def _iid_normal(n: int, dim: int, seed: int, device, d0: int, nd: int, layout: int, m: int) -> torch.Tensor:
    warnings.warn(f"{dim} base-sample dims exceed SobolEngine.MAXDIM={SOBOL_MAXDIM}: IID normal base samples",
                  RuntimeWarning)
    g = torch.Generator().manual_seed(int(seed))
    Z = torch.randn(n, dim, generator=g, dtype=torch.float64)[:, d0:d0 + nd]
    if layout == 0:
        return Z.contiguous().to(device)
    return Z.reshape(n, nd // m, m).permute(2, 1, 0).contiguous().to(device)


def sobol_scramble(dim: int, seed: int, d0: int = 0, nd: Optional[int] = None):
    nd = dim - d0 if nd is None else nd
    if not (0 <= d0 and nd >= 1 and d0 + nd <= dim):
        raise ValueError("sobol_scramble: dims out of range")
    if dim > SOBOL_MAXDIM:
        return None
    V, shift = _pinned_scramble_out(dim, d0, nd)
    call("evr_sobol_scramble_range", dim, int(seed), d0, nd, V.data_ptr(), shift.data_ptr())
    return V, shift


def _pinned_scramble_out(dim: int, d0: int, nd: int):
    pin = os.environ.get("EVR_SOBOL_PINNED", "1") != "0" and torch.cuda.is_available()
    V = torch.empty(nd, 30, dtype=torch.long, pin_memory=pin)
    V.copy_(_sobol_directions(dim)[d0:d0 + nd])
    return V, torch.empty(nd, dtype=torch.long, pin_memory=pin)


class SobolStream:

    def __init__(self, seed: int, max_dim: int):
        lib = _native.load()
        self._lib = lib
        self.seed, self.max_dim = int(seed), int(max_dim)
        h = ctypes.c_void_p()
        call("evr_sobol_stream_create", self.seed, lib.evr_sobol_stream_words(self.max_dim), ctypes.byref(h))
        self._h = h

    def scramble(self, dim: int, d0: int = 0, nd: Optional[int] = None):
        nd = dim - d0 if nd is None else nd
        if dim > SOBOL_MAXDIM or dim > self.max_dim or nd < 1:
            return None
        V, shift = _pinned_scramble_out(dim, d0, nd)
        call("evr_sobol_scramble_stream", self._h, dim, d0, nd, V.data_ptr(), shift.data_ptr())
        return V, shift

    def __del__(self):
        h = getattr(self, "_h", None)
        if h is not None:
            try:
                self._lib.evr_sobol_stream_destroy(h)
            except Exception:
                pass
            self._h = None


def sobol_normal(n: int, dim: int, seed: int, device, d0: int = 0, nd: Optional[int] = None,
                 layout: int = 0, m: int = 1, scrambled=None) -> torch.Tensor:
    nd = dim - d0 if nd is None else nd
    if not (0 <= d0 and d0 + nd <= dim):
        raise ValueError("sobol_normal: dims out of range")
    if dim > SOBOL_MAXDIM:
        return _iid_normal(n, dim, seed, device, d0, nd, layout, m)
    if layout == 0:
        out = torch.empty(n, nd, dtype=torch.float64, device=device)
    else:
        out = torch.empty(m, nd // m, n, dtype=torch.float64, device=device)
    if nd == 0:
        return out
    V, shift = scrambled if scrambled is not None else sobol_scramble(dim, seed, d0, nd)
    Vd = V.to(device, non_blocking=V.is_pinned())
    sd = shift.to(device, non_blocking=shift.is_pinned())
    call("evr_sobol_normal", _stream(), n, nd, 0, Vd.data_ptr(), sd.data_ptr(), layout, m, out.data_ptr())
    return out


def box_decompose(obj: np.ndarray, ref: np.ndarray, mask: Optional[np.ndarray] = None, num_threads: int = 0,
                  layout: str = "jis", alpha: float = 0.0):
    lib = _native.load()
    obj = np.ascontiguousarray(obj, dtype=np.float64)
    if layout == "jis":
        m, n, S = obj.shape
        ss, si, sj = 1, S, n * S
    elif layout == "sij":
        S, n, m = obj.shape
        ss, si, sj = n * m, m, 1
    else:
        raise ValueError(layout)
    ref = np.ascontiguousarray(ref, dtype=np.float64)
    mk = None if mask is None else np.ascontiguousarray(mask, dtype=np.uint8)
    handle = ctypes.c_void_p()
    _native.check(lib.evr_box_decompose_approx(S, n, m, obj.ctypes.data, ss, si, sj,
                                               None if mk is None else mk.ctypes.data, ref.ctypes.data,
                                               float(alpha), int(num_threads), ctypes.byref(handle)),
                  "evr_box_decompose_approx")
    try:
        total = lib.evr_cells_total(handle)
        lo = np.empty((total, m), dtype=np.float64)
        hi = np.empty((total, m), dtype=np.float64)
        off = np.empty(S + 1, dtype=np.int32)
        lib.evr_cells_copy(handle, lo.ctypes.data, hi.ctypes.data, off.ctypes.data)
    finally:
        lib.evr_cells_free(handle)
    return lo, hi, off


def device_arch(device: int = 0) -> str:
    buf = ctypes.create_string_buffer(64)
    call("evr_device_arch", device, buf, 64)
    return buf.value.decode()
```

include/everest_amd.h:

```cpp
#ifndef EVEREST_AMD_H
#define EVEREST_AMD_H

#ifdef __cplusplus
extern "C" {
#endif

#define EVR_VERSION 1

#define EVR_KERNEL_RBF 0
#define EVR_KERNEL_MATERN05 1
#define EVR_KERNEL_MATERN15 2
#define EVR_KERNEL_MATERN25 3
#define EVR_KERNEL_MIXED 16

int evr_version(void);
const char* evr_last_error(void);
int evr_device_arch(int device, char* buf, int buflen);
int evr_stream_sync(void* stream);

int evr_kernel_matrix(void* stream, int kind, int B, int n1, int n2, int d,
                      const double* X1, const double* shift1, const double* scale1,
                      const double* X2, const double* shift2, const double* scale2,
                      const double* lengthscales, const double* outputscale,
                      const double* diag_add, double* K);
// ... 53 lines not shown
                         int* info);

int evr_trsm_lower(void* stream, int batch, int n, int nrhs, const double* L, int ldl,
                   long long strideL, int transpose, double* B, int ldb, long long strideB);
int evr_tri_inv_lower(void* stream, int batch, int n, const double* L, int ldl, long long strideL,
                      double* Linv, int ldi, long long strideI);

int evr_gp_posterior_finalize(void* stream, int B, int n, int nt, const double* R,
                              const double* c, const double* ym, const double* ys,
                              const double* kxx, const double* noise_add,
                              double* mean, double* var);

long long evr_gp_posterior_workspace_doubles(int B, int n, int nt);
int evr_gp_posterior(void* stream, int B, int n, int nt, int d, int kind, const double* Xn, const double* X,
                     const double* shift, const double* scale, const double* lengthscales, const double* M,
                     const double* c, const double* ym, const double* ys, const double* kxx,
                     const double* noise_add, double* mean, double* var, double* work);

typedef struct {
  int n, nb, S, m;
  const double* c;
  const double* ym;
  const double* ys;
  const double* kxx;
  const double* zq;
  const double* obj_a;
  const double* obj_b;
  const double* cell_lo;
  const double* cell_hi;
  const int* cell_off;
  int max_cells;
  const unsigned long long* cell_keys;
  const double* cell_pts;
  const int* cell_rank0;
  int pts_stride;
  const int* grp_off;
  const unsigned long long* grp_keys;
  const unsigned short* grp_rank;
  const unsigned short* grp_box;
  const double* sorted_lo;
  int max_groups;
  unsigned long long* scan_counters;
  int no_h;
  int log_hvi;
  double tau_relu, tau_max;
} evr_qnehvi_state;

int evr_qnehvi_samples(void* stream, const evr_qnehvi_state* st, int b, const double* R,
                       double* G, double* L22, int* flags);
long long evr_hvi_workspace_doubles(const evr_qnehvi_state* st, int b, int backward);
int evr_hvi_forward(void* stream, const evr_qnehvi_state* st, int b, const double* G,
                    const int* flags, double* work, double* acq);
int evr_mean_over_samples(void* stream, int S, int b, const double* partial, double* acq);
int evr_hvi_backward(void* stream, const evr_qnehvi_state* st, int b, const double* G,
                     const double* gout, double* work, double* dG);
int evr_hvi_forward_backward(void* stream, const evr_qnehvi_state* st, int b, const double* G,
                             const int* flags, const double* gout, double* work, double* acq,
                             double* dG);
int evr_hvi_restart_fb_applies(const evr_qnehvi_state* st, int b);
int evr_hvi_scan_limits(int stride, int m);
int evr_hvi_restart_fb(void* stream, const evr_qnehvi_state* st, int b, const double* G, double* sval,
                       double* dG);
int evr_qnehvi_samples_backward(void* stream, const evr_qnehvi_state* st, int b, const double* R,
                                const double* L22, const double* dG, double* gR);

int evr_qnehvi_norms_rows(const evr_qnehvi_state* st);
int evr_qnehvi_project(void* stream, const evr_qnehvi_state* st, int b, const double* M, const double* Kx,
                       double* R, double* norms, double* work);
long long evr_qnehvi_project_workspace_doubles(const evr_qnehvi_state* st, int b);
int evr_qnehvi_samples_norms(void* stream, const evr_qnehvi_state* st, int b, const double* R,
                             const double* norms, double* G, double* L22, int* flags);
int evr_qnehvi_project_backward(void* stream, const evr_qnehvi_state* st, int b, const double* M,
                                const double* R, const double* L22, const double* dG, double* dKx,
                                double* work);
long long evr_qnehvi_project_backward_workspace_doubles(const evr_qnehvi_state* st, int b);

typedef struct {
  int n, d, kind;
  const double* Xn;
  const double* lengthscales;
  const double* shift;
  const double* scale;
  const double* M;
} evr_qnehvi_model;
typedef struct evr_qnehvi_plan evr_qnehvi_plan;
long long evr_qnehvi_plan_workspace_bytes(const evr_qnehvi_state* st, const evr_qnehvi_model* md, int b,
                                          int backward);
int evr_qnehvi_plan_create(void* stream, const evr_qnehvi_state* st, const evr_qnehvi_model* md, int b,
                           int backward, const double* X, void* work, double* acq, double* dX, int use_graph,
                           evr_qnehvi_plan** out);
int evr_qnehvi_small_applies(const evr_qnehvi_state* st, int b, int d);
long long evr_qnehvi_small_workspace_doubles(const evr_qnehvi_state* st, int b, int d, int which);
int evr_qnehvi_small_forward(void* stream, const evr_qnehvi_state* st, const evr_qnehvi_model* md, int b,
                             const double* Kx, double* R, double* P);
int evr_qnehvi_small_samples(void* stream, const evr_qnehvi_state* st, int b, const double* R, const double* P,
                             double* G, double* L22, int* flags);
int evr_qnehvi_small_backward(void* stream, const evr_qnehvi_state* st, const evr_qnehvi_model* md, int b,
                              const double* X, const double* R, const double* L22, const double* dG, double* dXp,
                              double* dX);
int evr_qnehvi_plan_run(void* stream, evr_qnehvi_plan* plan);
int evr_qnehvi_plan_eval_host(void* stream, evr_qnehvi_plan* plan, const double* x, double* out);
void evr_qnehvi_plan_destroy(evr_qnehvi_plan* plan);

#define EVR_LBFGSB_FG 1
#define EVR_LBFGSB_NEW_X 2
#define EVR_LBFGSB_CONV_PGTOL 3
#define EVR_LBFGSB_CONV_FACTR 4
#define EVR_LBFGSB_ABNORMAL 5
#define EVR_LBFGSB_ERROR 6
typedef struct evr_lbfgsb evr_lbfgsb;
int evr_lbfgsb_create(int n, int m, const double* lb, const double* ub, double factr, double pgtol, int maxls,
                      evr_lbfgsb** out);
int evr_lbfgsb_start(evr_lbfgsb* h, const double* x0, double* x);
int evr_lbfgsb_step(evr_lbfgsb* h, double f, const double* g, double* x);
void evr_lbfgsb_stats(const evr_lbfgsb* h, int* nit, int* nfev, double* f, double* pgnorm);
void evr_lbfgsb_destroy(evr_lbfgsb* h);

int evr_hit_and_run(int d, int rows, const double* A, const double* b, int k, const double* N,
                    const double* x0, long long n, unsigned long long seed, long long n_burnin,
                    long long n_thinning, double* out);

#define EVR_ERR_NOTPSD 7
int evr_qnehvi_plan_minimize(void* stream, evr_qnehvi_plan* plan, const double* x0, const double* lb,
                             const double* ub, int maxiter, int maxfun, double factr, double pgtol, int m,
                             int maxls, double* x, double* acq, int* info);

#define EVR_OBJ_AFFINE 0
#define EVR_OBJ_CLOSE_TO_TARGET 1
#define EVR_QNG_MAX_Q 12
typedef struct {
  int q;
  int m_obj;
  const int* obj_out;
  const int* obj_kind;
  const double* obj_p0;
  const double* obj_p1;
  int n_con;
  const int* con_out;
  const double* con_sign;
  const double* con_thr;
  const double* con_eta;
  const double* zq;
} evr_qn_general;
long long evr_qng_workspace_doubles(const evr_qnehvi_state* stm, const evr_qnehvi_state* sth,
                                    const evr_qn_general* g, const evr_qnehvi_model* md, int b, int backward);
int evr_qng_eval(void* stream, const evr_qnehvi_state* stm, const evr_qnehvi_state* sth, const evr_qn_general* g,
                 const evr_qnehvi_model* md, int b, const double* X, const double* gout, double* work,
                 double* acq, double* dX);
long long evr_qlog_workspace_doubles(const evr_qnehvi_state* stm, const evr_qnehvi_state* sth, const evr_qn_general* g,
                                     const evr_qnehvi_model* md, int b, int backward);
int evr_qlog_eval(void* stream, const evr_qnehvi_state* stm, const evr_qnehvi_state* sth, const evr_qn_general* g,
                  const evr_qnehvi_model* md, int b, const double* X, const double* gout, double* work,
                  double* acq, double* dX);
int evr_objective_general(void* stream, int m_model, int n, int S, const evr_qn_general* g, const double* Y,
                          const double* mu, const double* ref, double* O);
int evr_objective_weights(void* stream, int m_model, int n, const evr_qn_general* g, const double* Y, double* G,
                          double* W);

int evr_nei_scan(void* stream, int q, int log, int S, int b, const double* Y, const double* best,
                 int best_stride, double obj_a, double obj_b, double tau_relu, double tau_max,
                 const int* flags, const double* gout, double* acq, double* dY);
typedef struct {
  int log;
  double tau_relu;
  double tau_max;
  const double* best;
  int best_stride;
} evr_nei;
long long evr_qnei_workspace_doubles(const evr_qnehvi_state* stm, const evr_qn_general* g,
                                     const evr_qnehvi_model* md, int b, int backward);
int evr_qnei_eval(void* stream, const evr_qnehvi_state* stm, const evr_qn_general* g, const evr_qnehvi_model* md,
                  const evr_nei* nei, int b, const double* X, const double* gout, double* work, double* acq,
                  double* dX);

#define EVR_OBJ_SIGMOID 2
#define EVR_OBJ_TARGET 3
#define EVR_SOBO_MAX_TERMS 8
typedef struct {
  int log;
  double tau_relu;
  double tau_max;
  const double* best;
  int best_stride;
  int n_term;
  const int* term_out;
  const int* term_kind;
  const double* term_w;
  const double* term_p0;
  const double* term_p1;
  const double* term_p2;
  int n_con;
  const int* con_out;
  const double* con_sign;
  const double* con_thr;
  const double* con_eta;
} evr_sobo;
int evr_sobo_scan(void* stream, int q, int m_model, int S, int b, const evr_sobo* sb, const double* Y,
                  const int* flags, const double* gout, double* acq, double* dY);
long long evr_qsobo_workspace_doubles(const evr_qnehvi_state* stm, const evr_qn_general* g,
                                      const evr_qnehvi_model* md, int b, int backward);
int evr_qsobo_eval(void* stream, const evr_qnehvi_state* stm, const evr_qn_general* g, const evr_qnehvi_model* md,
                   const evr_sobo* sb, int b, const double* X, const double* gout, double* work, double* acq,
                   double* dX);

typedef struct {
  int log;
  double tau_relu;
  double tau_max;
  const double* best;
  int best_stride;
  double alpha;
  int n_term;
  const int* term_out;
  const int* term_kind;
  const double* term_p0;
  const double* term_p1;
  const double* term_a;
  const double* term_b;
  int n_con;
  const int* con_out;
  const double* con_sign;
  const double* con_thr;
  const double* con_eta;
} evr_parego;
int evr_parego_scan(void* stream, int q, int m_model, int S, int b, const evr_parego* pg, const double* Y,
                    const int* flags, const double* gout, double* acq, double* dY);
long long evr_qparego_workspace_doubles(const evr_qnehvi_state* stm, const evr_qn_general* g,
                                        const evr_qnehvi_model* md, int b, int backward);
int evr_qparego_eval(void* stream, const evr_qnehvi_state* stm, const evr_qn_general* g, const evr_qnehvi_model* md,
                     const evr_parego* pg, int b, const double* X, const double* gout, double* work, double* acq,
                     double* dX);

#define EVR_REWARD_SR 0
#define EVR_REWARD_UCB 1
#define EVR_REWARD_PI 2
typedef struct {
  int mode;
  double ucb_scale;
  double tau;
  const double* best;
  double infeasible_cost;
  int n_term;
  const int* term_out;
  const int* term_kind;
  const double* term_w;
  const double* term_p0;
  const double* term_p1;
  const double* term_p2;
  int n_con;
  const int* con_out;
  const double* con_sign;
  const double* con_thr;
  const double* con_eta;
} evr_reward;
int evr_reward_scan(void* stream, int q, int m_model, int S, int b, const evr_reward* rw, const double* Y,
                    const int* flags, const double* gout, double* acq, double* dY);
long long evr_qreward_workspace_doubles(const evr_qnehvi_state* stm, const evr_qn_general* g,
                                        const evr_qnehvi_model* md, int b, int backward);
int evr_qreward_eval(void* stream, const evr_qnehvi_state* stm, const evr_qn_general* g, const evr_qnehvi_model* md,
                     const evr_reward* rw, int b, const double* X, const double* gout, double* work, double* acq,
                     double* dX);

typedef struct {
  int log;
  double tau_relu;
  double tau_max;
  const double* best;
  int best_stride;
  int n_fac;
  const int* fac_out;
  const int* fac_kind;
  const double* fac_w;
  const double* fac_p0;
  const double* fac_p1;
  const double* fac_p2;
  int n_add;
  const int* add_out;
  const int* add_kind;
  const double* add_w;
  const double* add_p0;
  const double* add_p1;
  const double* add_p2;
} evr_mult;
int evr_mult_scan(void* stream, int q, int m_model, int S, int b, const evr_mult* mt, const double* Y,
                  const int* flags, const double* gout, double* acq, double* dY);
long long evr_qmult_workspace_doubles(const evr_qnehvi_state* stm, const evr_qn_general* g,
                                      const evr_qnehvi_model* md, int b, int backward);
int evr_qmult_eval(void* stream, const evr_qnehvi_state* stm, const evr_qn_general* g, const evr_qnehvi_model* md,
                   const evr_mult* mt, int b, const double* X, const double* gout, double* work, double* acq,
                   double* dX);

int evr_nipv_reduce(void* stream, int q, int B, int n, int N, int b, int d, int kind, const double* C,
                    const double* Vx, int ldv, const double* X, const double* lo, const double* inv_range,
                    const double* ls, const double* noise, const double* coef, const double* v0,
                    const double* gout, double* acq, int* flags, double* dC, double* dVx, double* dXself);


int evr_qei(void* stream, int n, int b, int S, const double* R, double c, double ym, double ys,
            double kxx, const double* z, double obj_a, double obj_b, double best_f, double* acq,
            double* gR, int* flags);

int evr_pareto_mask(void* stream, int S, int n, int m, const double* O, const double* ref,
                    int dedup, unsigned char* mask, int* counts);

int evr_objective_affine(void* stream, int m, int n, int S, const double* Y, const double* mu,
                         const double* a, const double* b, double* O);
int evr_scale_batched(void* stream, int B, long long per, const double* alpha, double* X);
int evr_add_selection(void* stream, int B, int nb, int n, const int* idx, const double* val, double* E);

typedef struct evr_cells evr_cells;
int evr_box_decompose(int S, int n, int m, const double* obj, long long ss, long long si,
                      long long sj, const unsigned char* mask, const double* ref, int num_threads,
                      evr_cells** out);
int evr_box_decompose_approx(int S, int n, int m, const double* obj, long long ss, long long si,
                             long long sj, const unsigned char* mask, const double* ref, double alpha,
                             int num_threads, evr_cells** out);
long long evr_cells_total(const evr_cells* c);
int evr_cells_copy(const evr_cells* c, double* lo, double* hi, int* off);
void evr_cells_free(evr_cells* c);

int evr_box_device_limits(int n, int m, int* max_points, long long* lds_bytes);
long long evr_box_device_workspace_bytes(int S, int n, int m, int cap);
int evr_box_decompose_device(void* stream, int S, int n, int m, const double* obj, const double* ref,
                             int cap, void* work, int* counts, int* status);
int evr_box_pack_keys_device(void* stream, int S, int n, int m, int cap, const void* work,
                             const int* off, int max_cells, unsigned long long* keys, double* pts,
                             int* rank0);
int evr_cells_from_keys(void* stream, int S, int m, int stride, const int* off, int max_cells,
                        const unsigned long long* keys, const double* pts, const int* rank0,
                        double* lo, double* hi);

int evr_box_kd_pipeline(void* stream, int S, int n, int m, const double* obj, const double* ref, int cap,
                        void* work, int* counts_dev, int* status_dev, int* off_dev, int* goff_dev,
                        unsigned long long* keys, double* pts, int* rank0, int want_kd, unsigned long long* okeys,
                        unsigned short* ork, unsigned short* ogb, double* osv, int* counts_host, int* info);
int evr_cells_kd_limits(int stride, int m, int max_cells, long long* lds_bytes);
int evr_cells_kd_order_device(void* stream, int S, int m, int stride, const int* off, const int* goff,
                              int max_cells, const unsigned long long* keys, const double* pts,
                              const int* rank0, unsigned long long* okeys, unsigned short* ork,
                              unsigned short* ogb, double* osv);

int evr_sobol_scramble(int dim, unsigned long long seed, long long* V, long long* shift);
int evr_sobol_scramble_range(int dim, unsigned long long seed, int d0, int nd, long long* V, long long* shift);
typedef struct evr_sobol_stream evr_sobol_stream;
long long evr_sobol_stream_words(int dim);
int evr_sobol_stream_create(unsigned long long seed, long long nwords, evr_sobol_stream** out);
int evr_sobol_scramble_stream(const evr_sobol_stream* st, int dim, int d0, int nd, long long* V, long long* shift);
void evr_sobol_stream_destroy(evr_sobol_stream* st);
int evr_sobol_normal(void* stream, int n, int nd, int d0, const long long* V, const long long* shift,
                     int layout, int m, double* out);

#ifdef __cplusplus
}
#endif
#endif
```

Before: 204,000 candidates/s.

## Split device box decomposition into begin/finish so launch happens on caller thread

The kd box-decomposition pipeline is split into a begin step, which enqueues the decomposition kernel on a side stream from the calling thread, and a finish step, which the worker thread runs after waiting on an event. Per-call staging buffers and events move into pooled tickets instead of thread_local state, so several decompositions can be in flight at once. This is meant to start GPU work earlier and remove the Python-thread handoff latency from the critical path. It also adds a Pareto sort-key kernel and helper. The cost is more complex lifetime management, with a risk of leaked tickets or races if finish is skipped.

```diff
diff --git a/everest_amd/_native.py b/everest_amd/_native.py
--- a/everest_amd/_native.py
+++ b/everest_amd/_native.py
@@ -132,6 +132,7 @@
     "evr_qnehvi_samples_backward": ([c_void_p, POINTER(EvrQnehviState), c_int, c_void_p, c_void_p, c_void_p,
                                      c_void_p], c_int),
     "evr_pareto_mask": ([c_void_p, c_int, c_int, c_int, c_void_p, c_void_p, c_int, c_void_p, c_void_p], c_int),
+    "evr_pareto_sort_key": ([c_int, c_void_p], ctypes.c_uint),
     "evr_objective_affine": ([c_void_p, c_int, c_int, c_int] + [c_void_p] * 5, c_int),
     "evr_qei": ([c_void_p, c_int, c_int, c_int, c_void_p, c_double, c_double, c_double, c_double, c_void_p,
                  c_double, c_double, c_double, c_void_p, c_void_p, c_void_p], c_int),
@@ -152,6 +153,9 @@
                                   c_void_p, c_void_p], c_int),
     "evr_box_kd_pipeline": ([c_void_p, c_int, c_int, c_int, c_void_p, c_void_p, c_int] + [c_void_p] * 8
                             + [c_int] + [c_void_p] * 6, c_int),
+    "evr_box_kd_begin": ([c_void_p, c_void_p, c_int, c_int, c_int, c_void_p, c_void_p, c_int, c_void_p, c_void_p,
+                          c_void_p, c_int, POINTER(c_void_p)], c_int),
+    "evr_box_kd_finish": ([c_void_p] * 6 + [c_int] + [c_void_p] * 6, c_int),
     "evr_cells_from_keys": ([c_void_p, c_int, c_int, c_int, c_void_p, c_int] + [c_void_p] * 5, c_int),
     "evr_hvi_forward_backward": ([c_void_p, POINTER(EvrQnehviState), c_int] + [c_void_p] * 6, c_int),
     "evr_hvi_restart_fb_applies": ([POINTER(EvrQnehviState), c_int], c_int),
diff --git a/everest_amd/acquisition.py b/everest_amd/acquisition.py
--- a/everest_amd/acquisition.py
+++ b/everest_amd/acquisition.py
@@ -85,18 +85,30 @@
                      hi=torch.full((S, m), math.inf, dtype=torch.float64, device=dev))
 
 
+def _device_box(O: torch.Tensor, box_device, alpha: float) -> bool:
+    m, P, _ = O.shape
+    return not (alpha > 0.0 and m > 2) and bool(
+        box_device if box_device is not None else
+        ops.box_device_supported(P, m) and ops.hvi_scan_supported(P + m, m))
+
+
+def _box_pipeline(kd_scan) -> bool:
+    return kd_scan is not False and os.environ.get("EVR_BOX_PIPELINE", "1") != "0"
+
+
 def _decompose(O: torch.Tensor, ref: torch.Tensor, box_device=None, kd_scan=None, num_threads=None,
-               alpha: float = 0.0):
+               alpha: float = 0.0, started: Optional[ops.BoxKdPending] = None):
     m, P, _ = O.shape
     dev = O.device
     approx = alpha > 0.0 and m > 2
     if approx and box_device:
         raise ValueError("the device box decomposition is exact only (alpha = 0)")
-    if not approx and (box_device if box_device is not None else
-                       ops.box_device_supported(P, m) and ops.hvi_scan_supported(P + m, m)):
+    if _device_box(O, box_device, alpha):
         kd_built = False
         try:
-            if kd_scan is False or os.environ.get("EVR_BOX_PIPELINE", "1") == "0":
+            if started is not None:
+                cells, kd_built = ops.box_decompose_kd_finish(started)
+            elif not _box_pipeline(kd_scan):
                 cells = ops.box_decompose_device(O, ref)
             else:
                 cells, kd_built = ops.box_decompose_kd_device(O, ref, want_kd=True)
@@ -132,8 +144,10 @@
 _SIDE_STREAMS = {}
 
 
-def _decompose_async(O: torch.Tensor, ref: torch.Tensor, *args):
+def _decompose_async(O: torch.Tensor, ref: torch.Tensor, box_device=None, kd_scan=None, num_threads=None,
+                     alpha: float = 0.0):
     global _BOX_POOL
+    args = (box_device, kd_scan, num_threads, alpha)
     if os.environ.get("EVR_BOX_OVERLAP", "1") == "0" or not O.is_cuda:
         res = _decompose(O, ref, *args)
         return lambda: res
@@ -142,10 +156,18 @@
     side = _SIDE_STREAMS.get(dev)
     if side is None:
         side = _SIDE_STREAMS[dev] = torch.cuda.Stream(dev)
-    ready = torch.cuda.Event()
-    ready.record(main)
-    O.record_stream(side)
-    ref.record_stream(side)
+    started = None
+    if _device_box(O, box_device, alpha) and _box_pipeline(kd_scan):
+        try:
+            started = ops.box_decompose_kd_begin(O, ref, want_kd=True, stream=side)
+        except ops.BoxCapacityError:
+            pass
+    ready = None
+    if started is None:
+        ready = torch.cuda.Event()
+        ready.record(main)
+        O.record_stream(side)
+        ref.record_stream(side)
     if _BOX_POOL is None:
         from concurrent.futures import ThreadPoolExecutor
 
@@ -153,8 +175,9 @@
 
     def job():
         with torch.cuda.device(dev), torch.cuda.stream(side):
-            side.wait_event(ready)
-            return _decompose(O, ref, *args)
+            if ready is not None:
+                side.wait_event(ready)
+            return _decompose(O, ref, *args, started=started)
 
     fut = _BOX_POOL.submit(job)
 
diff --git a/everest_amd/csrc/box_device.hip b/everest_amd/csrc/box_device.hip
--- a/everest_amd/csrc/box_device.hip
+++ b/everest_amd/csrc/box_device.hip
@@ -1,6 +1,8 @@
 #include <algorithm>
 #include <cmath>
 #include <cstdlib>
+#include <mutex>
+#include <vector>
 
 #include "common.hpp"
 #include "../../include/everest_amd.h"
@@ -363,15 +365,15 @@
 }
 
 static int box_decompose_launch(void* stream, int S, int n, int m, const double* obj, const double* ref, int cap,
-                                void* work, int* counts, int* status, int* hmap);
+                                void* work, int* counts, int* status, int* hmap, int lds_slab);
 
 int evr_box_decompose_device(void* stream, int S, int n, int m, const double* obj, const double* ref, int cap,
                              void* work, int* counts, int* status) {
-  return box_decompose_launch(stream, S, n, m, obj, ref, cap, work, counts, status, nullptr);
+  return box_decompose_launch(stream, S, n, m, obj, ref, cap, work, counts, status, nullptr, -1);
 }
 
 static int box_decompose_launch(void* stream, int S, int n, int m, const double* obj, const double* ref, int cap,
-                                void* work, int* counts, int* status, int* hmap) {
+                                void* work, int* counts, int* status, int* hmap, int lds_slab) {
   EVR_CHECK(S >= 1 && n >= 1 && m >= 1 && m <= 8 && obj && ref && work && counts && status,
             "evr_box_decompose_device: bad arguments");
   EVR_CHECK(cap >= 2 && (cap & (cap - 1)) == 0, "evr_box_decompose_device: cap must be a power of two");
@@ -385,8 +387,11 @@
     return c;
   };
   const size_t fixed_ls = fixed + (size_t)BD_STG * (8 + 4);
-  const char* ev = std::getenv("EVR_BD_LDS");
-  const bool ls = sort_cap(fixed_ls) >= cap && !(ev && ev[0] == '0');
+  if (lds_slab < 0) {
+    const char* ev = std::getenv("EVR_BD_LDS");
+    lds_slab = !(ev && ev[0] == '0');
+  }
+  const bool ls = sort_cap(fixed_ls) >= cap && lds_slab;
   const int sortcap = ls ? cap : sort_cap(fixed);
   const size_t lds = (ls ? fixed_ls : fixed) + (size_t)sortcap * 8;
   hipStream_t s = (hipStream_t)stream;
@@ -438,44 +443,104 @@
 }
 
 
-int evr_box_kd_pipeline(void* stream, int S, int n, int m, const double* obj, const double* ref, int cap,
-                        void* work, int* counts_dev, int* status_dev, int* off_dev, int* goff_dev,
-                        unsigned long long* keys, double* pts, int* rank0, int want_kd, unsigned long long* okeys,
-                        unsigned short* ork, unsigned short* ogb, double* osv, int* counts_host, int* info) {
-  EVR_CHECK(S >= 1 && counts_dev && status_dev && off_dev && goff_dev && keys && pts && rank0 && counts_host &&
-                info && (!want_kd || (okeys && ork && ogb && osv)),
-            "evr_box_kd_pipeline: bad arguments");
-  hipStream_t s = (hipStream_t)stream;
-  thread_local int* stage = nullptr;
-  thread_local int* stage_d = nullptr;
-  thread_local size_t stage_n = 0;
-  thread_local int stage_dev = -1;
-  thread_local hipEvent_t copied = nullptr;
-  if (copied) EVR_HIP(hipEventSynchronize(copied));
-  int dev = 0;
-  EVR_HIP(hipGetDevice(&dev));
-  const size_t need = (size_t)4 * S + 2;
-  if (stage_n < need || stage_dev != dev) {
-    if (copied) {
-      (void)hipEventDestroy(copied);
-      copied = nullptr;
-    }
-    if (stage) (void)hipHostFree(stage);
-    stage = stage_d = nullptr;
-    stage_n = 0;
-    stage_dev = -1;
-    EVR_HIP(hipHostMalloc((void**)&stage, sizeof(int) * need, hipHostMallocMapped | hipHostMallocCoherent));
-    EVR_HIP(hipHostGetDevicePointer((void**)&stage_d, stage, 0));
-    stage_n = need;
-    stage_dev = dev;
-  }
-  if (!copied) EVR_HIP(hipEventCreateWithFlags(&copied, hipEventDisableTiming));
-  int* hc = stage;
-  int* hs = stage + S;
-  int* hoff = stage + 2 * S;
+namespace {
+
+struct BoxTicket {
+  int dev = -1;
+  int* stage = nullptr;
+  int* stage_d = nullptr;
+  size_t stage_n = 0;
+  hipEvent_t ready = nullptr;
+  hipEvent_t built = nullptr;
+  hipEvent_t copied = nullptr;
+  bool copied_set = false;
+  hipStream_t s = nullptr;
+  int S = 0, n = 0, m = 0, cap = 0;
+  const void* work = nullptr;
+};
+
+std::mutex g_ticket_mu;
+std::vector<BoxTicket*> g_tickets;
+
+void ticket_release(BoxTicket* t) {
+  std::lock_guard<std::mutex> lk(g_ticket_mu);
+  g_tickets.push_back(t);
+}
+
+void ticket_destroy(BoxTicket* t) {
+  if (t->copied_set) (void)hipEventSynchronize(t->copied);
+  if (t->ready) (void)hipEventDestroy(t->ready);
+  if (t->built) (void)hipEventDestroy(t->built);
+  if (t->copied) (void)hipEventDestroy(t->copied);
+  if (t->stage) (void)hipHostFree(t->stage);
+  delete t;
+}
+
+int ticket_acquire(int dev, size_t need, BoxTicket** out) {
+  BoxTicket* t = nullptr;
+  {
+    std::lock_guard<std::mutex> lk(g_ticket_mu);
+    for (size_t i = 0; i < g_tickets.size(); ++i)
+      if (g_tickets[i]->dev == dev && g_tickets[i]->stage_n >= need) {
+        t = g_tickets[i];
+        g_tickets.erase(g_tickets.begin() + i);
+        break;
+      }
+    if (!t)
+      for (size_t i = 0; i < g_tickets.size(); ++i)
+        if (g_tickets[i]->dev == dev) {
+          ticket_destroy(g_tickets[i]);
+          g_tickets.erase(g_tickets.begin() + i);
+          break;
+        }
+  }
+  if (!t) {
+    t = new BoxTicket();
+    t->dev = dev;
+    bool ok = hipHostMalloc((void**)&t->stage, sizeof(int) * need, hipHostMallocMapped | hipHostMallocCoherent) ==
+                  hipSuccess &&
+              hipHostGetDevicePointer((void**)&t->stage_d, t->stage, 0) == hipSuccess &&
+              hipEventCreateWithFlags(&t->ready, hipEventDisableTiming) == hipSuccess &&
+              hipEventCreateWithFlags(&t->built, hipEventDisableTiming) == hipSuccess &&
+              hipEventCreateWithFlags(&t->copied, hipEventDisableTiming) == hipSuccess;
+    if (!ok) {
+      (void)hipGetLastError();
+      ticket_destroy(t);
+      EVR_CHECK(false, "evr_box_kd_begin: cannot allocate %zu B of mapped host staging", sizeof(int) * need);
+    }
+    t->stage_n = need;
+  }
+  *out = t;
+  return 0;
+}
+
+int box_kd_begin(BoxTicket* t, void* after_stream, const double* obj, const double* ref, int* counts_dev,
+                 int* status_dev, int flags) {
+  hipStream_t s = t->s;
+  if (after_stream != (void*)s) {
+    EVR_HIP(hipEventRecord(t->ready, (hipStream_t)after_stream));
+    EVR_HIP(hipStreamWaitEvent(s, t->ready, 0));
+  }
+  if (t->copied_set) EVR_HIP(hipStreamWaitEvent(s, t->copied, 0));
+  if (int rc = box_decompose_launch((void*)s, t->S, t->n, t->m, obj, ref, t->cap, (void*)t->work, counts_dev,
+                                    status_dev, t->stage_d, (flags & 1) ? 0 : 1))
+    return rc;
+  EVR_HIP(hipEventRecord(t->built, s));
+  EVR_HIP(hipEventRecord(t->copied, s));
+  t->copied_set = true;
+  return 0;
+}
+
+int box_kd_finish(BoxTicket* t, int* off_dev, int* goff_dev, unsigned long long* keys, double* pts, int* rank0,
+                  int want_kd, unsigned long long* okeys, unsigned short* ork, unsigned short* ogb, double* osv,
+                  int* counts_host, int* info) {
+  const int S = t->S, n = t->n, m = t->m, cap = t->cap;
+  hipStream_t s = t->s;
+  int* hc = t->stage;
+  int* hs = t->stage + S;
+  int* hoff = t->stage + 2 * S;
   int* hgoff = hoff + S + 1;
-  if (int rc = box_decompose_launch(stream, S, n, m, obj, ref, cap, work, counts_dev, status_dev, stage_d)) return rc;
-  EVR_HIP(hipStreamSynchronize(s));
+  EVR_HIP(hipEventSynchronize(t->built));
   info[0] = info[1] = info[2] = 0;
   int maxc = 0;
   for (int i = 0; i < S; ++i) {
@@ -494,21 +559,77 @@
   }
   hoff[S] = (int)c;
   hgoff[S] = (int)g;
-  EVR_CHECK(c <= (long long)S * cap && c < 0x7FFFFFFFLL, "evr_box_kd_pipeline: %lld cells exceed the capacity", c);
-  const int* moff = stage_d + 2 * S;
+  EVR_CHECK(c <= (long long)S * cap && c < 0x7FFFFFFFLL, "evr_box_kd_finish: %lld cells exceed the capacity", c);
+  const int* moff = t->stage_d + 2 * S;
   const int* mgoff = moff + S + 1;
-  if (int rc = evr_box_pack_keys_device(stream, S, n, m, cap, work, moff, maxc, keys, pts, rank0)) return rc;
+  if (int rc = evr_box_pack_keys_device((void*)s, S, n, m, cap, t->work, moff, maxc, keys, pts, rank0)) return rc;
   const int stride = n + m;
   if (want_kd && evr_cells_kd_limits(stride, m, maxc, nullptr) == 0) {
-    if (int rc = evr_cells_kd_order_device(stream, S, m, stride, moff, mgoff, maxc, keys, pts, rank0, okeys, ork,
+    if (int rc = evr_cells_kd_order_device((void*)s, S, m, stride, moff, mgoff, maxc, keys, pts, rank0, okeys, ork,
                                            ogb, osv))
       return rc;
     info[1] = 1;
   }
   EVR_HIP(hipMemcpyAsync(off_dev, hoff, sizeof(int) * (S + 1), hipMemcpyHostToDevice, s));
   EVR_HIP(hipMemcpyAsync(goff_dev, hgoff, sizeof(int) * (S + 1), hipMemcpyHostToDevice, s));
-  EVR_HIP(hipEventRecord(copied, s));
+  EVR_HIP(hipEventRecord(t->copied, s));
   return 0;
 }
 
 }
+
+int evr_box_kd_begin(void* stream, void* after_stream, int S, int n, int m, const double* obj, const double* ref,
+                     int cap, void* work, int* counts_dev, int* status_dev, int flags, void** ticket) {
+  EVR_CHECK(S >= 1 && counts_dev && status_dev && ticket, "evr_box_kd_begin: bad arguments");
+  *ticket = nullptr;
+  int dev = 0;
+  EVR_HIP(hipGetDevice(&dev));
+  BoxTicket* t = nullptr;
+  if (int rc = ticket_acquire(dev, (size_t)4 * S + 2, &t)) return rc;
+  t->s = (hipStream_t)stream;
+  t->S = S, t->n = n, t->m = m, t->cap = cap;
+  t->work = work;
+  if (int rc = box_kd_begin(t, after_stream, obj, ref, counts_dev, status_dev, flags)) {
+    ticket_release(t);
+    return rc;
+  }
+  *ticket = t;
+  return 0;
+}
+
+int evr_box_kd_finish(void* ticket, int* off_dev, int* goff_dev, unsigned long long* keys, double* pts, int* rank0,
+                      int want_kd, unsigned long long* okeys, unsigned short* ork, unsigned short* ogb, double* osv,
+                      int* counts_host, int* info) {
+  EVR_CHECK(ticket, "evr_box_kd_finish: no ticket");
+  BoxTicket* t = (BoxTicket*)ticket;
+  int rc = 2;
+  if (off_dev && goff_dev && keys && pts && rank0 && counts_host && info && (!want_kd || (okeys && ork && ogb && osv))) {
+    int cur = t->dev;
+    (void)hipGetDevice(&cur);
+    if (cur != t->dev) (void)hipSetDevice(t->dev);
+    rc = box_kd_finish(t, off_dev, goff_dev, keys, pts, rank0, want_kd, okeys, ork, ogb, osv, counts_host, info);
+    if (cur != t->dev) (void)hipSetDevice(cur);
+  } else {
+    ::evr::set_error("evr_box_kd_finish: bad arguments");
+  }
+  ticket_release(t);
+  return rc;
+}
+
+int evr_box_kd_pipeline(void* stream, int S, int n, int m, const double* obj, const double* ref, int cap,
+                        void* work, int* counts_dev, int* status_dev, int* off_dev, int* goff_dev,
+                        unsigned long long* keys, double* pts, int* rank0, int want_kd, unsigned long long* okeys,
+                        unsigned short* ork, unsigned short* ogb, double* osv, int* counts_host, int* info) {
+  EVR_CHECK(S >= 1 && counts_dev && status_dev && off_dev && goff_dev && keys && pts && rank0 && counts_host &&
+                info && (!want_kd || (okeys && ork && ogb && osv)),
+            "evr_box_kd_pipeline: bad arguments");
+  const char* ev = std::getenv("EVR_BD_LDS");
+  void* ticket = nullptr;
+  if (int rc = evr_box_kd_begin(stream, stream, S, n, m, obj, ref, cap, work, counts_dev, status_dev,
+                                (ev && ev[0] == '0') ? 1 : 0, &ticket))
+    return rc;
+  return evr_box_kd_finish(ticket, off_dev, goff_dev, keys, pts, rank0, want_kd, okeys, ork, ogb, osv, counts_host,
+                           info);
+}
+
+}
diff --git a/everest_amd/csrc/qnehvi.hip b/everest_amd/csrc/qnehvi.hip
--- a/everest_amd/csrc/qnehvi.hip
+++ b/everest_amd/csrc/qnehvi.hip
@@ -1,5 +1,6 @@
 #include <algorithm>
 #include <cstdlib>
+#include <cstring>
 #include <string>
 #include "common.hpp"
 #include "../../include/everest_amd.h"
@@ -295,6 +296,151 @@
   }
 }
 
+__host__ __device__ inline unsigned int pareto_key_word(const float* f, int m) {
+  float key = f[0];
+  for (int j = 1; j < m; ++j) key = key + f[j];
+  key = key + 0.0f;
+  if (key != key) return 0u;
+  unsigned int b;
+  memcpy(&b, &key, sizeof b);
+  const unsigned int asc = b ^ ((b >> 31) ? 0xFFFFFFFFu : 0x80000000u);
+  return ~asc;
+}
+
+constexpr int PS_THREADS = 512;
+
+template <int M>
+__global__ __launch_bounds__(PS_THREADS) void pareto_sorted_kernel(int S, int n, int npad, int npow, int SB,
+                                                                   const double* __restrict__ O,
+                                                                   const double* __restrict__ ref, int dedup,
+                                                                   unsigned char* __restrict__ mask,
+                                                                   int* __restrict__ counts) {
+  extern __shared__ unsigned long long srt[];
+  float* ptf = reinterpret_cast<float*>(srt + (((size_t)SB * npow + 1) & ~(size_t)1));
+  unsigned short* inv = reinterpret_cast<unsigned short*>(ptf + (size_t)SB * M * npad);
+  const int s0 = blockIdx.x * SB, sb = min(SB, S - s0);
+  const int tid = threadIdx.x;
+  double rj[M];
+#pragma unroll
+  for (int j = 0; j < M; ++j) rj[j] = ref[j];
+  for (int e = tid; e < sb * npow; e += PS_THREADS) {
+    const int k = e / sb, ss = e - k * sb;
+    unsigned long long w = ~0ull;
+    if (k < n) {
+      float f[M];
+      bool better = true;
+#pragma unroll
+      for (int j = 0; j < M; ++j) {
+        const double v = O[((size_t)j * n + k) * S + s0 + ss];
+        better &= v > rj[j];
+        f[j] = (float)v;
+      }
+      w = ((unsigned long long)pareto_key_word(f, M) << 32) | (better ? 0u : 0x80000000u) | (unsigned int)k;
+    }
+    srt[(size_t)ss * npow + k] = w;
+  }
+  __syncthreads();
+  const int half = npow >> 1;
+  for (int kk = 2; kk <= npow; kk <<= 1)
+    for (int jj = kk >> 1; jj > 0; jj >>= 1) {
+      for (int e = tid; e < sb * half; e += PS_THREADS) {
+        const int ss = e / half, t = e - ss * half;
+        const int i = ((t & ~(jj - 1)) << 1) | (t & (jj - 1));
+        unsigned long long* A = srt + (size_t)ss * npow;
+        const unsigned long long a = A[i], b = A[i + jj];
+        if ((a > b) == ((i & kk) == 0)) {
+          A[i] = b;
+          A[i + jj] = a;
+        }
+      }
+      __syncthreads();
+    }
+  for (int e = tid; e < sb * n; e += PS_THREADS) {
+    const int ss = e / n, r = e - ss * n;
+    inv[(size_t)ss * npow + ((unsigned int)srt[(size_t)ss * npow + r] & 0x7FFFFFFFu)] = (unsigned short)r;
+  }
+  for (int e = tid; e < sb * M * (npad - n); e += PS_THREADS) {
+    const int r = e / (npad - n), k = n + (e - r * (npad - n));
+    ptf[(size_t)r * npad + k] = -INFINITY;
+  }
+  __syncthreads();
+  for (int e = tid; e < sb * n; e += PS_THREADS) {
+    const int k = e / sb, ss = e - k * sb;
+    const int r = inv[(size_t)ss * npow + k];
+#pragma unroll
+    for (int j = 0; j < M; ++j)
+      ptf[((size_t)ss * M + j) * npad + r] = (float)O[((size_t)j * n + k) * S + s0 + ss];
+  }
+  __syncthreads();
+  for (int p = tid; p < sb * n; p += PS_THREADS) {
+    const int ss = p / n, q = p - ss * n;
+    const int r = (ss & 1) ? n - 1 - q : q;
+    const unsigned long long* A = srt + (size_t)ss * npow;
+    const float* F = ptf + (size_t)ss * M * npad;
+    const unsigned long long wi = A[r];
+    const int i = (int)((unsigned int)wi & 0x7FFFFFFFu);
+    const unsigned int hi = (unsigned int)(wi >> 32), bound = hi ? hi : 0xFFFFFFFFu;
+    float yf[M];
+#pragma unroll
+    for (int j = 0; j < M; ++j) yf[j] = F[(size_t)j * npad + r];
+    bool nd = !((unsigned int)wi >> 31);
+    bool have = false;
+    double yi[M];
+    for (int k0 = 0; k0 < n && nd && (unsigned int)(A[k0] >> 32) <= bound; k0 += 8) {
+      float4 va[M], vb[M];
+#pragma unroll
+      for (int j = 0; j < M; ++j) {
+        va[j] = *reinterpret_cast<const float4*>(F + (size_t)j * npad + k0);
+        vb[j] = *reinterpret_cast<const float4*>(F + (size_t)j * npad + k0 + 4);
+      }
+      bool ge8[8];
+#pragma unroll
+      for (int u = 0; u < 8; ++u) ge8[u] = k0 + u != r && k0 + u < n;
+#pragma unroll
+      for (int j = 0; j < M; ++j) {
+        ge8[0] &= va[j].x >= yf[j]; ge8[1] &= va[j].y >= yf[j];
+        ge8[2] &= va[j].z >= yf[j]; ge8[3] &= va[j].w >= yf[j];
+        ge8[4] &= vb[j].x >= yf[j]; ge8[5] &= vb[j].y >= yf[j];
+        ge8[6] &= vb[j].z >= yf[j]; ge8[7] &= vb[j].w >= yf[j];
+      }
+      unsigned int cand = 0;
+#pragma unroll
+      for (int u = 0; u < 8; ++u) cand |= (unsigned int)ge8[u] << u;
+      while (cand) {
+        const int u = __builtin_ctz(cand);
+        cand &= cand - 1;
+        bool strict = true;
+#pragma unroll
+        for (int j = 0; j < M; ++j) strict &= F[(size_t)j * npad + k0 + u] > yf[j];
+        if (strict) {
+          nd = false;
+          break;
+        }
+        if (!have) {
+#pragma unroll
+          for (int j = 0; j < M; ++j) yi[j] = O[((size_t)j * n + i) * S + s0 + ss];
+          have = true;
+        }
+        const int k = (int)((unsigned int)A[k0 + u] & 0x7FFFFFFFu);
+        bool ge = true, gt = false, eq = true;
+#pragma unroll
+        for (int j = 0; j < M; ++j) {
+          const double v = O[((size_t)j * n + k) * S + s0 + ss];
+          ge &= v >= yi[j];
+          gt |= v > yi[j];
+          eq &= v == yi[j];
+        }
+        if ((ge && gt) || (dedup && eq && k < i)) {
+          nd = false;
+          cand = 0;
+        }
+      }
+    }
+    if (mask) mask[(size_t)(s0 + ss) * n + i] = nd ? 1 : 0;
+    if (counts && nd) atomicAdd(&counts[i], 1);
+  }
+}
+
 __global__ void qei_kernel(int n, int b, int S, const double* __restrict__ R, double cc, double ym, double ys,
                            double kxx, const double* __restrict__ z, double oa, double ob, double best_f,
                            double* __restrict__ acq, double* __restrict__ gR, int* __restrict__ flags) {
@@ -435,8 +581,29 @@
   hipStream_t s = (hipStream_t)stream;
   constexpr size_t kLds = 96 * 1024;
   const size_t per = (size_t)n * m * sizeof(double);
+  const int npad = (n + 7) & ~7;
+  constexpr size_t kLds3 = 78 * 1024;
+  int npow = 1;
+  while (npow < n) npow *= 2;
+  const size_t per3 = (size_t)npow * (sizeof(unsigned long long) + sizeof(unsigned short)) +
+                      (size_t)npad * m * sizeof(float);
+  if (per3 + 8 <= kLds3 && n < 65536) {
+    const int SB = (int)std::min<size_t>(4, (kLds3 - 8) / per3);
+    const size_t bytes = (((size_t)SB * npow + 1) & ~(size_t)1) * sizeof(unsigned long long) +
+                         (size_t)SB * npad * m * sizeof(float) + (size_t)SB * npow * sizeof(unsigned short);
+#define L(MM)                                                                                          \
+  do {                                                                                                 \
+    EVR_HIP(hipFuncSetAttribute((const void*)pareto_sorted_kernel<MM>,                                  \
+                                hipFuncAttributeMaxDynamicSharedMemorySize, (int)bytes));              \
+    pareto_sorted_kernel<MM><<<cdiv(S, SB), PS_THREADS, bytes, s>>>(S, n, npad, npow, SB, O, ref, dedup, \
+                                                                    mask, counts);                     \
+  } while (0)
+    EVR_DISPATCH_M(m, L);
+#undef L
+    EVR_LAUNCH_CHECK();
+    return 0;
+  }
   constexpr int f32_filter = 1;
-  const int npad = (n + 7) & ~7;
   const size_t per2 = (size_t)n * m * sizeof(double) + (size_t)npad * m * sizeof(float);
   constexpr size_t kLds2 = 78 * 1024;
   if (f32_filter && per2 <= kLds2) {
@@ -471,6 +638,13 @@
   return 0;
 }
 
+unsigned int evr_pareto_sort_key(int m, const double* y) {
+  float f[8];
+  if (!y || m < 1 || m > 8) return 0u;
+  for (int j = 0; j < m; ++j) f[j] = (float)y[j];
+  return pareto_key_word(f, m);
+}
+
 int evr_qei(void* stream, int n, int b, int S, const double* R, double c, double ym, double ys, double kxx,
             const double* z, double obj_a, double obj_b, double best_f, double* acq, double* gR, int* flags) {
   EVR_CHECK(n >= 1 && S >= 1, "evr_qei: bad sizes");
diff --git a/everest_amd/ops.py b/everest_amd/ops.py
--- a/everest_amd/ops.py
+++ b/everest_amd/ops.py
@@ -1192,61 +1192,124 @@
     return Cells(off, counts, m, keys=keys, pts=pts, rank0=rank0, stride=stride)
 
 
+def _box_kd_buffers(S: int, n: int, m: int, cap: int, want_kd: bool, dev, max_workspace_bytes: int) -> dict:
+    stride = n + m
+    nbytes = _native.load().evr_box_device_workspace_bytes(S, n, m, cap)
+    G = S * cap // 16 + S
+    out_bytes = 8 * S * cap + 8 * S * stride * m + 4 * S * stride + 16 * S + 8
+    if want_kd:
+        out_bytes += G * 16 * 8 + G * m * 16 * 2 + G * 8 * 2 + 8 * S * m * stride
+    if nbytes + out_bytes > max_workspace_bytes:
+        raise BoxCapacityError(f"box decomposition: {cap} LUB slots x {S} samples need {nbytes + out_bytes} B "
+                               "of workspace and outputs")
+    try:
+        b = dict(ws=torch.empty(nbytes, dtype=torch.uint8, device=dev),
+                 cs=torch.empty(2, S, dtype=torch.int32, device=dev),
+                 offs=torch.empty(2, S + 1, dtype=torch.int32, device=dev),
+                 keys=torch.empty(S * cap, dtype=torch.int64, device=dev),
+                 pts=torch.empty(S, stride, m, dtype=torch.float64, device=dev),
+                 rank0=torch.empty(S, stride, dtype=torch.int32, device=dev),
+                 okeys=None, ork=None, ogb=None, osv=None)
+        if want_kd:
+            b.update(okeys=torch.empty(G * 16, dtype=torch.int64, device=dev),
+                     ork=torch.empty(G * m * 16, dtype=torch.int16, device=dev),
+                     ogb=torch.empty(G * 8, dtype=torch.int16, device=dev),
+                     osv=torch.empty(S, m, stride, dtype=torch.float64, device=dev))
+    except torch.OutOfMemoryError as e:
+        raise BoxCapacityError(f"box decomposition: out of device memory at {cap} LUB slots x {S} samples") from e
+    return b
+
+
+def _box_kd_cells(b: dict, counts_h: np.ndarray, info: np.ndarray, S: int, n: int, m: int, copy: bool):
+    counts = counts_h.astype(np.int64)
+    total = int(counts.sum())
+    trim = (lambda t: t.clone()) if copy else (lambda t: t)
+    cells = Cells(b["offs"][0], counts, m, keys=trim(b["keys"][:max(total, 1)]), pts=b["pts"], rank0=b["rank0"],
+                  stride=n + m)
+    if info[1]:
+        ng = (counts + 15) // 16
+        Gu = int(ng.sum())
+        cells.kd = KdGroups(b["offs"][1], trim(b["okeys"][:max(Gu, 1) * 16]), trim(b["ork"][:max(Gu, 1) * m * 16]),
+                            trim(b["ogb"][:max(Gu, 1) * 8]), b["osv"], int(ng.max()) if S else 0)
+    return cells, bool(info[1])
+
+
 def box_decompose_kd_device(O: torch.Tensor, ref: torch.Tensor, want_kd: bool = True, cap: int = 16384,
-                            max_cap: int = 1 << 20, max_workspace_bytes: int = 8 << 30):
+                            max_cap: int = 1 << 20, max_workspace_bytes: int = 8 << 30, _cap0: Optional[int] = None):
     O, ref = _dev(O, "O"), _dev(ref, "ref")
     m, n, S = O.shape
-    dev = O.device
-    stride = n + m
-    lib = _native.load()
     counts_h = np.zeros(S, dtype=np.int32)
     info = np.zeros(3, dtype=np.int32)
-    cap0 = cap
+    cap0 = cap if _cap0 is None else _cap0
     while True:
-        nbytes = lib.evr_box_device_workspace_bytes(S, n, m, cap)
-        G = S * cap // 16 + S
-        out_bytes = 8 * S * cap + 8 * S * stride * m + 4 * S * stride + 16 * S + 8
-        if want_kd:
-            out_bytes += G * 16 * 8 + G * m * 16 * 2 + G * 8 * 2 + 8 * S * m * stride
-        if nbytes + out_bytes > max_workspace_bytes:
-            raise BoxCapacityError(f"box decomposition: {cap} LUB slots x {S} samples need {nbytes + out_bytes} B "
-                                   "of workspace and outputs")
-        try:
-            ws = torch.empty(nbytes, dtype=torch.uint8, device=dev)
-            cs = torch.empty(2, S, dtype=torch.int32, device=dev)
-            offs = torch.empty(2, S + 1, dtype=torch.int32, device=dev)
-            keys = torch.empty(S * cap, dtype=torch.int64, device=dev)
-            pts = torch.empty(S, stride, m, dtype=torch.float64, device=dev)
-            rank0 = torch.empty(S, stride, dtype=torch.int32, device=dev)
-            if want_kd:
-                okeys = torch.empty(G * 16, dtype=torch.int64, device=dev)
-                ork = torch.empty(G * m * 16, dtype=torch.int16, device=dev)
-                ogb = torch.empty(G * 8, dtype=torch.int16, device=dev)
-                osv = torch.empty(S, m, stride, dtype=torch.float64, device=dev)
-            else:
-                okeys = ork = ogb = osv = None
-        except torch.OutOfMemoryError as e:
-            raise BoxCapacityError(f"box decomposition: out of device memory at {cap} LUB slots x {S} samples") from e
-        call("evr_box_kd_pipeline", _stream(), S, n, m, O.data_ptr(), ref.data_ptr(), cap, ws.data_ptr(),
-             cs[0].data_ptr(), cs[1].data_ptr(), offs[0].data_ptr(), offs[1].data_ptr(), keys.data_ptr(),
-             pts.data_ptr(), rank0.data_ptr(), int(bool(want_kd)), _p(okeys), _p(ork), _p(ogb), _p(osv),
-             counts_h.ctypes.data, info.ctypes.data)
+        b = _box_kd_buffers(S, n, m, cap, want_kd, O.device, max_workspace_bytes)
+        call("evr_box_kd_pipeline", _stream(), S, n, m, O.data_ptr(), ref.data_ptr(), cap, b["ws"].data_ptr(),
+             b["cs"][0].data_ptr(), b["cs"][1].data_ptr(), b["offs"][0].data_ptr(), b["offs"][1].data_ptr(),
+             b["keys"].data_ptr(), b["pts"].data_ptr(), b["rank0"].data_ptr(), int(bool(want_kd)), _p(b["okeys"]),
+             _p(b["ork"]), _p(b["ogb"]), _p(b["osv"]), counts_h.ctypes.data, info.ctypes.data)
         if not info[0]:
             break
         if cap >= max_cap:
             raise BoxCapacityError(f"box decomposition: more than {max_cap} local upper bounds in one sample")
         cap *= 4
-    counts = counts_h.astype(np.int64)
-    total = int(counts.sum())
-    del ws
-    trim = (lambda t: t.clone()) if cap > cap0 else (lambda t: t)
-    cells = Cells(offs[0], counts, m, keys=trim(keys[:max(total, 1)]), pts=pts, rank0=rank0, stride=stride)
-    if info[1]:
-        ng = (counts + 15) // 16
-        Gu = int(ng.sum())
-        cells.kd = KdGroups(offs[1], trim(okeys[:max(Gu, 1) * 16]), trim(ork[:max(Gu, 1) * m * 16]),
-                            trim(ogb[:max(Gu, 1) * 8]), osv, int(ng.max()) if S else 0)
-    return cells, bool(info[1])
+    return _box_kd_cells(b, counts_h, info, S, n, m, copy=cap > cap0)
+
+
+class BoxKdPending:
+
+    def __init__(self, O, ref, want_kd, cap, max_cap, max_workspace_bytes, stream, buffers, ticket):
+        self.O, self.ref, self.want_kd, self.cap, self.max_cap = O, ref, want_kd, cap, max_cap
+        self.max_workspace_bytes, self.stream, self.buffers, self.ticket = max_workspace_bytes, stream, buffers, ticket
+
+    def __del__(self):
+        if getattr(self, "ticket", None):
+            try:
+                _native.load().evr_box_kd_finish(self.ticket, *([None] * 5), 0, *([None] * 6))
+            except Exception:
+                pass
+            self.ticket = None
+
+
+def box_decompose_kd_begin(O: torch.Tensor, ref: torch.Tensor, want_kd: bool = True, cap: int = 16384,
+                           max_cap: int = 1 << 20, max_workspace_bytes: int = 8 << 30,
+                           stream: Optional[torch.cuda.Stream] = None) -> BoxKdPending:
+    O, ref = _dev(O, "O"), _dev(ref, "ref")
+    m, n, S = O.shape
+    cur = torch.cuda.current_stream(O.device)
+    stream = cur if stream is None else stream
+    with torch.cuda.device(O.device), torch.cuda.stream(stream):
+        b = _box_kd_buffers(S, n, m, cap, want_kd, O.device, max_workspace_bytes)
+    if stream != cur:
+        O.record_stream(stream)
+        ref.record_stream(stream)
+    ticket = ctypes.c_void_p()
+    with torch.cuda.device(O.device):
+        call("evr_box_kd_begin", stream.cuda_stream, cur.cuda_stream, S, n, m, O.data_ptr(), ref.data_ptr(), cap,
+             b["ws"].data_ptr(), b["cs"][0].data_ptr(), b["cs"][1].data_ptr(),
+             1 if os.environ.get("EVR_BD_LDS", "1")[:1] == "0" else 0, ctypes.byref(ticket))
+    return BoxKdPending(O, ref, want_kd, cap, max_cap, max_workspace_bytes, stream, b, ticket)
+
+
+def box_decompose_kd_finish(p: BoxKdPending):
+    if not p.ticket:
+        raise RuntimeError("box_decompose_kd_finish: already finished")
+    m, n, S = p.O.shape
+    b = p.buffers
+    counts_h = np.zeros(S, dtype=np.int32)
+    info = np.zeros(3, dtype=np.int32)
+    ticket, p.ticket = p.ticket, None
+    call("evr_box_kd_finish", ticket, b["offs"][0].data_ptr(), b["offs"][1].data_ptr(), b["keys"].data_ptr(),
+         b["pts"].data_ptr(), b["rank0"].data_ptr(), int(bool(p.want_kd)), _p(b["okeys"]), _p(b["ork"]), _p(b["ogb"]),
+         _p(b["osv"]), counts_h.ctypes.data, info.ctypes.data)
+    p.buffers = None
+    if not info[0]:
+        return _box_kd_cells(b, counts_h, info, S, n, m, copy=False)
+    if p.cap >= p.max_cap:
+        raise BoxCapacityError(f"box decomposition: more than {p.max_cap} local upper bounds in one sample")
+    b = None
+    with torch.cuda.device(p.O.device), torch.cuda.stream(p.stream):
+        return box_decompose_kd_device(p.O, p.ref, p.want_kd, p.cap * 4, p.max_cap, p.max_workspace_bytes,
+                                       _cap0=p.cap)
 
 
 _SOBOL_DIRECTIONS = {}
diff --git a/include/everest_amd.h b/include/everest_amd.h
--- a/include/everest_amd.h
+++ b/include/everest_amd.h
@@ -379,6 +379,7 @@
 
 int evr_pareto_mask(void* stream, int S, int n, int m, const double* O, const double* ref,
                     int dedup, unsigned char* mask, int* counts);
+unsigned int evr_pareto_sort_key(int m, const double* y);
 
 int evr_objective_affine(void* stream, int m, int n, int S, const double* Y, const double* mu,
                          const double* a, const double* b, double* O);
@@ -411,6 +412,11 @@
                         void* work, int* counts_dev, int* status_dev, int* off_dev, int* goff_dev,
                         unsigned long long* keys, double* pts, int* rank0, int want_kd, unsigned long long* okeys,
                         unsigned short* ork, unsigned short* ogb, double* osv, int* counts_host, int* info);
+int evr_box_kd_begin(void* stream, void* after_stream, int S, int n, int m, const double* obj, const double* ref,
+                     int cap, void* work, int* counts_dev, int* status_dev, int flags, void** ticket);
+int evr_box_kd_finish(void* ticket, int* off_dev, int* goff_dev, unsigned long long* keys, double* pts, int* rank0,
+                      int want_kd, unsigned long long* okeys, unsigned short* ork, unsigned short* ogb, double* osv,
+                      int* counts_host, int* info);
 int evr_cells_kd_limits(int stride, int m, int max_cells, long long* lds_bytes);
 int evr_cells_kd_order_device(void* stream, int S, int m, int stride, const int* off, const int* goff,
                               int max_cells, const unsigned long long* keys, const double* pts,
```

New measurement: 204,500 candidates/s (median of 2 runs). No clear change (+0.3%).
